# MariusFurter/WeightedSampling.jl

Measured on NVIDIA B200. Metric: particle_updates_per_sec, higher is better.
Workload: dtype f64

## Files before the change

weightedsampling.jl_b200/csrc/ws_internal.h:

```cpp
#pragma once
#include <cuda_runtime.h>
#include <stdint.h>
#include "ws_vm.cuh"
#include "ws_mailbox.cuh"

#ifndef WS_VM_BLOCK
#define WS_VM_BLOCK 128
#endif
#ifndef WS_VM_P
#define WS_VM_P 3
#endif
#ifndef WS_VM_MINB
#define WS_VM_MINB 5
#endif
#define WS_VM_MAX_IO 24
#define WS_VM_MAX_CKPT 16
#define WS_VM_MAX_OPS 96
#define WS_VM_MAX_REGS ((192 * 1024) / (WS_VM_BLOCK * WS_VM_P * 8))
#define WS_SCAN_BLOCK 256
#define WS_SCAN_ITEMS 8
#define WS_SCAN_TILE (32 * WS_SCAN_ITEMS)
#define WS_CDF_TILE (WS_SCAN_BLOCK * WS_SCAN_ITEMS)
#define WS_GATHER_MAX_PLANES 32
#define WS_HEAVY_TILE_SLOTS 32768
#define WS_MAX_PARTIALS 4096

struct WsLse {
    double m, S, Q;
};

struct WsReduceOut {
    double m, S, Q;
    double lse;
    double ess_perc;
    double log_mean_w;
    int32_t do_resample;
    int32_t pad;
};

struct WsVmProgram {
    int64_t n;
    int64_t particle_offset;
    int32_t n_ops, n_loads, n_stores, n_regs;
    const double* load_ptr[WS_VM_MAX_IO];
    double* store_ptr[WS_VM_MAX_IO];
    uint8_t load_reg[WS_VM_MAX_IO];
    uint8_t store_reg[WS_VM_MAX_IO];
    const int32_t* ancestors;
    uint32_t load_gather;
    int32_t logw_mode;
    double* logw;
    double logw_base;
    WsLse* partials;
    int32_t n_expect;
    uint8_t expect_reg[8];
    const WsReduceOut* red;
    double* expect_partials;
    int32_t n_ckpt;
    uint8_t ckpt_pc[WS_VM_MAX_CKPT];
    WsLse* ckpt_partials;
    double* logw_out;
    WsRng rng;
    WsOp ops[WS_VM_MAX_OPS];
};

struct WsScanParams {
    const double* logw;
    int32_t mode;
    int32_t scheme;
    const WsReduceOut* red;
    int32_t gate;
    int32_t pad;
    int64_t n;
    int64_t n_slots;
    unsigned long long cdf_offset;
    const unsigned long long* all_tot;
    int32_t rank;
    int32_t pad2;
    int32_t slot_base;
    int32_t last_rank;
    int32_t* bounds;
    unsigned long long* total;
    uint64_t seed, stream;
    const double* replay_u;
    const double* sorted_u;
    int32_t* ancestors;
    unsigned long long* tile_words;
    unsigned long long* cdf_local;
    unsigned int* tile_counter;
    double fx_scale;
    int32_t fx_shift;
    int32_t mn_shift;
    unsigned long long* mn_tile_off;
    unsigned long long* mn_block_local;
    unsigned long long* mn_total;
    unsigned long long* n_clamped;
    unsigned int* heavy_count;
    int32_t* heavy_F;
};

struct WsGatherParams {
    int64_t n;
    const int32_t* ancestors;
    int32_t n_planes;
    int32_t pad;
    const double* src[WS_GATHER_MAX_PLANES];
    double* dst[WS_GATHER_MAX_PLANES];
};

#define WS_COMPOSE_MAX_CHAIN 24
struct WsComposeParams {
    int64_t n;
    int64_t n_rows;
    int32_t n_chain;
    int32_t pad;
    const int32_t* chain[WS_COMPOSE_MAX_CHAIN];
};

cudaError_t ws_launch_vm(const WsVmProgram& P, int grid, cudaStream_t s);
cudaError_t ws_launch_reduce_logw(const double* logw, int64_t n, WsLse* partials, int grid, cudaStream_t s);
cudaError_t ws_launch_finalize(const WsLse* partials, int n_partials, int k, int64_t n_global, double ess_perc_min,
                               WsReduceOut* out, unsigned long long* ties, cudaStream_t s);
#define WS_SMALL_N 4096
cudaError_t ws_launch_resample_small(const WsScanParams& P, const WsLse* partials, int n_partials, double ess_perc_min, WsReduceOut* out,
                                     unsigned long long* ties, int do_finalize, cudaStream_t s);
void ws_scan_set_scale(WsScanParams& P);
size_t ws_scan_words(int64_t n);
cudaError_t ws_launch_scan_search(const WsScanParams& P, int grid, cudaStream_t s);
cudaError_t ws_launch_spacings(const WsScanParams& P, cudaStream_t s);
cudaError_t ws_launch_cdf(const WsScanParams& P, cudaStream_t s);
cudaError_t ws_launch_bounds(const WsScanParams& P, cudaStream_t s);
cudaError_t ws_launch_search(const WsScanParams& P, cudaStream_t s);
cudaError_t ws_launch_finalize_global(const double* all_msq, int n_ranks, int64_t n_global, double ess_perc_min,
                                      WsReduceOut* out, cudaStream_t s, unsigned long long* ties = nullptr);
cudaError_t ws_launch_finalize_mbox(const WsLse* partials, int n_partials, int64_t n_global, double ess_perc_min, WsReduceOut* out,
                                    double* all_msq, unsigned long long* ties, const WsMailbox& M, cudaStream_t s);
cudaError_t ws_launch_cdf_tiles(const WsScanParams& P, cudaStream_t s);
cudaError_t ws_launch_offsets_bounds_mbox(const WsScanParams& P, const WsMailbox& M, unsigned long long* all_tot, const unsigned long long* xmine,
                                          int xw, unsigned long long* xall, cudaStream_t s);
cudaError_t ws_launch_barrier_mbox(const WsMailbox& M, cudaStream_t s);
cudaError_t ws_launch_gather(const WsGatherParams& P, int grid, cudaStream_t s);
cudaError_t ws_launch_fill(double* dst, double v, int64_t n, int grid, cudaStream_t s);
cudaError_t ws_launch_exp_norm(const double* logw, const WsReduceOut* red, double* w, int64_t n, int grid,
                               cudaStream_t s);
cudaError_t ws_launch_sumsq(const double* w, int64_t n, double* partials, int grid, cudaStream_t s);
cudaError_t ws_launch_local_ancestors(int32_t* anc, int64_t n, const int32_t* anc_self, int64_t self_lo, int64_t self_hi,
                                      int64_t spare_base, int grid, cudaStream_t s);
cudaError_t ws_launch_patch_ancestors(int32_t* anc, int64_t n, int64_t self_lo, int64_t self_hi, int64_t spare_base, cudaStream_t s);
struct WsTracedPlane {
    const double* src;
    double* dst;
    int64_t level;
};
cudaError_t ws_launch_trace_rows(const int32_t* anc, int64_t m, const int32_t* const* chain, int n_levels, int64_t n_rows, int32_t* rows,
                                 cudaStream_t s);
cudaError_t ws_launch_push_traced(const WsTracedPlane* planes, int n_planes, int64_t m, const int32_t* rows, cudaStream_t s);
cudaError_t ws_launch_gather_rows(const double* src, const int64_t* idx, int64_t n_idx, double* dst, cudaStream_t s);
cudaError_t ws_launch_compose(const WsComposeParams& P, int32_t* out, const int32_t* start, cudaStream_t s);
cudaError_t ws_launch_compose_rows(const WsComposeParams& P, int64_t* out, const int64_t* start, cudaStream_t s);
int ws_vm_sl_grid(const WsVmProgram& P);
int ws_vm_max_grid(int n_regs, int n_loads, int n_ops, int sm_count, int n_ckpt = 0);
int ws_vm_smem_bytes(int n_regs, int n_loads, int n_ops, int n_ckpt = 0);
cudaError_t ws_kernels_init(int device);
```

weightedsampling.jl_b200/csrc/ws_kernels.cu:

```cuda
#include "ws_internal.h"

static int g_sm_count = 148;

__device__ __forceinline__ void lse_push(WsLse& a, double l) {
    if (l == -INFINITY) return;
    if (l > a.m) {
        double sc = ws_exp_nonpos(a.m - l);
        a.S = a.S * sc + 1.0;
        a.Q = a.Q * sc * sc + 1.0;
        a.m = l;
    } else {
        double e = ws_exp_nonpos(l - a.m);
        a.S += e;
        a.Q += e * e;
    }
}

template <int K>
__device__ __forceinline__ void lse_push_many(WsLse& a, const double (&l)[K], const bool (&live)[K]) {
    double mx = -INFINITY;
#pragma unroll
    for (int j = 0; j < K; ++j)
        if (live[j]) mx = fmax(mx, l[j]);
    if (mx > a.m) {
// ... 11 lines not shown
        }
    }
}

__device__ __forceinline__ WsLse lse_combine(const WsLse& a, const WsLse& b) {
    if (b.m == -INFINITY) return a;
    if (a.m == -INFINITY) return b;
    WsLse r;
    r.m = fmax(a.m, b.m);
    double ea = ws_exp_nonpos(a.m - r.m), eb = ws_exp_nonpos(b.m - r.m);
    r.S = a.S * ea + b.S * eb;
    r.Q = a.Q * ea * ea + b.Q * eb * eb;
    return r;
}

__device__ __forceinline__ WsLse lse_shfl_down(const WsLse& a, int delta) {
    WsLse r;
    r.m = __shfl_down_sync(0xffffffffu, a.m, delta);
    r.S = __shfl_down_sync(0xffffffffu, a.S, delta);
    r.Q = __shfl_down_sync(0xffffffffu, a.Q, delta);
    return r;
}

template <int BLOCK>
__device__ __forceinline__ WsLse lse_block_reduce(WsLse v, WsLse* warp_scratch ) {
#pragma unroll
    for (int d = 16; d > 0; d >>= 1) v = lse_combine(v, lse_shfl_down(v, d));
    const int lane = threadIdx.x & 31, warp = threadIdx.x >> 5;
    if (lane == 0) warp_scratch[warp] = v;
    __syncthreads();
    if (warp == 0) {
        WsLse t;
        if (lane < BLOCK / 32) {
            t = warp_scratch[lane];
        } else {
            t.m = -INFINITY;
            t.S = 0.0;
            t.Q = 0.0;
        }
#pragma unroll
        for (int d = 16; d > 0; d >>= 1) t = lse_combine(t, lse_shfl_down(t, d));
        v = t;
    }
    return v;
}

template <int BLOCK>
__device__ __forceinline__ WsLse lse_block_combine(const WsLse* __restrict__ partials, int n_partials, WsLse* warp_scratch ) {
    WsLse part;
    part.m = -INFINITY;
    part.S = 0.0;
    part.Q = 0.0;
    for (int i = threadIdx.x; i < n_partials; i += BLOCK) part = lse_combine(part, partials[i]);
    return lse_block_reduce<BLOCK>(part, warp_scratch);
}

__device__ __forceinline__ WsLse lse_combine_ranks(const double* msq, int n_ranks) {
    WsLse tot;
    tot.m = -INFINITY;
    tot.S = 0.0;
    tot.Q = 0.0;
    for (int r = 0; r < n_ranks; ++r) {
        WsLse v;
        v.m = msq[3 * r + 0];
        v.S = msq[3 * r + 1];
        v.Q = msq[3 * r + 2];
        tot = lse_combine(tot, v);
    }
    return tot;
}

__device__ __forceinline__ void ws_decide(const WsLse& tot, int64_t n_global, double ess_perc_min, WsReduceOut* out,
                                          unsigned long long* ties) {
    out->m = tot.m;
    out->S = tot.S;
    out->Q = tot.Q;
    const double lse = tot.m + log(tot.S);
    out->lse = lse;
    const double nn = (double)n_global;
    out->ess_perc = (tot.S * tot.S) / (nn * tot.Q);
    out->log_mean_w = lse - log(nn);
    out->do_resample = (out->ess_perc < ess_perc_min) ? 1 : 0;
    if (ties != nullptr && fabs(out->ess_perc - ess_perc_min) <= 8.0 * 2.220446049250313e-16 * fabs(ess_perc_min)) atomicAdd(ties, 1ull);
}

__device__ __forceinline__ void ws_cp_async8(double* smem_dst, const double* gsrc) {
    const unsigned d = (unsigned)__cvta_generic_to_shared(smem_dst);
    asm volatile("cp.async.ca.shared.global [%0], [%1], 8;" ::"r"(d), "l"(gsrc) : "memory");
}
__device__ __forceinline__ void ws_cp_async16(void* smem_dst, const void* gsrc) {
    const unsigned d = (unsigned)__cvta_generic_to_shared(smem_dst);
    asm volatile("cp.async.cg.shared.global [%0], [%1], 16;" ::"r"(d), "l"(gsrc) : "memory");
}
__device__ __forceinline__ void ws_cp_async_commit() { asm volatile("cp.async.commit_group;" ::: "memory"); }
__device__ __forceinline__ void ws_cp_async_wait_all() { asm volatile("cp.async.wait_group 0;" ::: "memory"); }

template <bool STAGED, bool CKPT = false>
__global__ void __launch_bounds__(WS_VM_BLOCK, WS_VM_MINB) ws_vm_kernel(const __grid_constant__ WsVmProgram P) {
    extern __shared__ __align__(16) double ws_vm_smem[];
    __shared__ WsLse warp_scratch[WS_VM_BLOCK / 32];
    double* R = ws_vm_smem + threadIdx.x;
    constexpr int RS = WS_VM_P * WS_VM_BLOCK;
    double* const stage = R + P.n_regs * RS;
    WsDop* const dops = reinterpret_cast<WsDop*>(ws_vm_smem + (P.n_regs + (STAGED ? P.n_loads : 0)) * RS);
    for (int t = threadIdx.x; t < P.n_ops; t += WS_VM_BLOCK) dops[t] = ws_decode_op<WS_VM_BLOCK, WS_VM_P>(P.ops[t]);
    double* const ck = reinterpret_cast<double*>(dops + P.n_ops) + threadIdx.x;
    for (int c = 0; CKPT && c < P.n_ckpt; ++c) {
        ck[(c * 3 + 0) * WS_VM_BLOCK] = -INFINITY;
        ck[(c * 3 + 1) * WS_VM_BLOCK] = 0.0;
        ck[(c * 3 + 2) * WS_VM_BLOCK] = 0.0;
    }
    __syncthreads();

    WsLse part;
    part.m = -INFINITY;
    part.S = 0.0;
    part.Q = 0.0;
    double esum[8];
#pragma unroll
    for (int k = 0; k < 8; ++k) esum[k] = 0.0;
    double red_m = 0.0, red_invS = 0.0;
    if (P.n_expect > 0) {
        red_m = P.red->m;
        red_invS = 1.0 / P.red->S;
    }

    constexpr int TILE = WS_VM_BLOCK * WS_VM_P;
    const int n = (int)P.n;
    const int n_tiles = (n + TILE - 1) / TILE;
    const bool fired = (P.logw_mode != 3) || P.red->do_resample != 0;
    const int lmode = (P.logw_mode == 3) ? (fired ? 2 : 1) : P.logw_mode;
    const double lbase = (P.logw_mode == 3) ? P.red->log_mean_w : P.logw_base;
    const bool any_gather = P.load_gather != 0u && fired;

    auto tile_index = [&](int tile, int j) -> int {
        const int i = tile * TILE + (int)threadIdx.x + j * WS_VM_BLOCK;
        return i < n ? i : n - 1;
    };
    auto issue_stage = [&](int tile, const int (&anc)[WS_VM_P]) {
        for (int k = 0; k < P.n_loads; ++k) {
            const bool g = any_gather && ((P.load_gather >> k) & 1u);
            const double* __restrict__ ptr = P.load_ptr[k];
            double* dst = stage + k * RS;
#pragma unroll
            for (int j = 0; j < WS_VM_P; ++j)
                ws_cp_async8(dst + j * WS_VM_BLOCK, ptr + (unsigned)(g ? anc[j] : tile_index(tile, j)));
        }
        ws_cp_async_commit();
    };

    int anc_next[WS_VM_P];
    if (STAGED) {
        const int t0 = blockIdx.x, t1 = blockIdx.x + gridDim.x;
        if (t0 < n_tiles) {
            int a0[WS_VM_P];
#pragma unroll
            for (int j = 0; j < WS_VM_P; ++j) a0[j] = any_gather ? __ldg(P.ancestors + tile_index(t0, j)) : 0;
            issue_stage(t0, a0);
        }
#pragma unroll
        for (int j = 0; j < WS_VM_P; ++j) anc_next[j] = (any_gather && t1 < n_tiles) ? __ldg(P.ancestors + tile_index(t1, j)) : 0;
    }

    for (int tile = blockIdx.x; tile < n_tiles; tile += gridDim.x) {
        int idx[WS_VM_P];
        bool live[WS_VM_P];
// ... 98 lines not shown
            const double* srcr = R + (int)P.store_reg[k] * RS;
            double* __restrict__ ptr = P.store_ptr[k];
#pragma unroll
            for (int j = 0; j < WS_VM_P; ++j)
                if (live[j]) ptr[(unsigned)idx[j]] = srcr[j * WS_VM_BLOCK];
        }
        if (P.logw_mode != 0) {
            double lw[WS_VM_P];
#pragma unroll
            for (int j = 0; j < WS_VM_P; ++j) {
                lw[j] = (CKPT ? lw_run[j] : (lmode == 1 ? lw_old[j] : lbase)) + acc[j];
                if (live[j]) (CKPT && P.logw_out != nullptr ? P.logw_out : P.logw)[(unsigned)idx[j]] = lw[j];
            }
            lse_push_many<WS_VM_P>(part, lw, live);
        }
        if (P.n_expect > 0) {
#pragma unroll
            for (int j = 0; j < WS_VM_P; ++j) {
                if (live[j]) {
                    const double w = ws_exp_nonpos(lw_old[j] - red_m) * red_invS;
#pragma unroll
                    for (int k = 0; k < 8; ++k) {
                        if (k < P.n_expect) esum[k] += w * R[(int)P.expect_reg[k] * RS + j * WS_VM_BLOCK];
                    }
                }
            }
        }
    }

    if (P.logw_mode != 0 && P.partials != nullptr) {
        WsLse tot = lse_block_reduce<WS_VM_BLOCK>(part, warp_scratch);
        if (threadIdx.x == 0) P.partials[blockIdx.x] = tot;
    }
    for (int c = 0; CKPT && c < P.n_ckpt; ++c) {
        WsLse st;
        st.m = ck[(c * 3 + 0) * WS_VM_BLOCK];
        st.S = ck[(c * 3 + 1) * WS_VM_BLOCK];
        st.Q = ck[(c * 3 + 2) * WS_VM_BLOCK];
        __syncthreads();
        WsLse tot = lse_block_reduce<WS_VM_BLOCK>(st, warp_scratch);
        if (threadIdx.x == 0) P.ckpt_partials[(size_t)c * gridDim.x + blockIdx.x] = tot;
    }
    if (P.n_expect > 0) {
        __shared__ double esc[WS_VM_BLOCK / 32][8];
        const int lane = threadIdx.x & 31, warp = threadIdx.x >> 5;
#pragma unroll
        for (int k = 0; k < 8; ++k) {
            double v = esum[k];
#pragma unroll
            for (int d = 16; d > 0; d >>= 1) v += __shfl_down_sync(0xffffffffu, v, d);
            if (lane == 0) esc[warp][k] = v;
        }
        __syncthreads();
        if (threadIdx.x < 8 && threadIdx.x < P.n_expect) {
            double v = 0.0;
            for (int w = 0; w < WS_VM_BLOCK / 32; ++w) v += esc[w][threadIdx.x];
            P.expect_partials[(size_t)blockIdx.x * P.n_expect + threadIdx.x] = v;
        }
    }
}

#include "ws_vm_sl.cuh"
#ifndef WS_SL_P
#define WS_SL_P 4
#endif
#ifndef WS_SL_MINB
#define WS_SL_MINB 3
#endif
template <class Sig, int PP>
__global__ void __launch_bounds__(WS_VM_BLOCK, WS_SL_MINB) ws_vm_sl_kernel(const __grid_constant__ WsVmProgram P) {
    extern __shared__ __align__(16) double ws_vm_smem[];
    __shared__ WsLse warp_scratch[WS_VM_BLOCK / 32];
    constexpr int RS = PP * WS_VM_BLOCK;
    constexpr int TILE = WS_VM_BLOCK * PP;
    constexpr int NL = Sig::n_loads, NS = Sig::n_stores;
    double* const stage = ws_vm_smem + threadIdx.x;

    WsLse part;
    part.m = -INFINITY;
    part.S = 0.0;
    part.Q = 0.0;
    const int n = (int)P.n;
    const int n_tiles = (n + TILE - 1) / TILE;
    const bool fired = (P.logw_mode != 3) || P.red->do_resample != 0;
    const int lmode = (P.logw_mode == 3) ? (fired ? 2 : 1) : P.logw_mode;
    const double lbase = (P.logw_mode == 3) ? P.red->log_mean_w : P.logw_base;
    const bool any_gather = P.load_gather != 0u && fired;

    auto tile_index = [&](int tile, int j) -> int {
        const int i = tile * TILE + (int)threadIdx.x + j * WS_VM_BLOCK;
        return i < n ? i : n - 1;
    };
    auto issue_stage = [&](int tile, const int (&anc)[PP]) {
#pragma unroll
        for (int k = 0; k < NL; ++k) {
            const bool g = any_gather && ((P.load_gather >> k) & 1u);
            const double* __restrict__ ptr = P.load_ptr[k];
#pragma unroll
            for (int j = 0; j < PP; ++j)
                ws_cp_async8(stage + k * RS + j * WS_VM_BLOCK, ptr + (unsigned)(g ? anc[j] : tile_index(tile, j)));
        }
        ws_cp_async_commit();
    };

    WsSlConsts<Sig> K;
    ws_sl_load_consts<Sig>(K, P, std::make_integer_sequence<int, Sig::n_ops>{});
    const bool replay = P.rng.replay_n != nullptr || P.rng.replay_u != nullptr || P.rng.replay_e != nullptr;

    int anc_next[PP];
    {
        const int t0 = blockIdx.x, t1 = blockIdx.x + gridDim.x;
        if (t0 < n_tiles) {
            int a0[PP];
#pragma unroll
            for (int j = 0; j < PP; ++j) a0[j] = any_gather ? __ldg(P.ancestors + tile_index(t0, j)) : 0;
            issue_stage(t0, a0);
        }
#pragma unroll
        for (int j = 0; j < PP; ++j) anc_next[j] = (any_gather && t1 < n_tiles) ? __ldg(P.ancestors + tile_index(t1, j)) : 0;
    }

    for (int tile = blockIdx.x; tile < n_tiles; tile += gridDim.x) {
        int idx[PP];
        bool live[PP];
        uint64_t particle[PP];
        const int first = tile * TILE + (int)threadIdx.x;
#pragma unroll
        for (int j = 0; j < PP; ++j) {
            const int i = first + j * WS_VM_BLOCK;
            live[j] = i < n;
            idx[j] = live[j] ? i : n - 1;
            particle[j] = (uint64_t)(P.particle_offset + (int64_t)idx[j]);
        }
        double R[Sig::n_regs * PP];
        if (NL > 0) {
            ws_cp_async_wait_all();
            ws_sl_loads<Sig, PP, WS_VM_BLOCK>(R, stage, std::make_integer_sequence<int, NL>{});
            const int tn = tile + gridDim.x, tnn = tn + gridDim.x;
            if (tn < n_tiles) issue_stage(tn, anc_next);
            if (any_gather && tnn < n_tiles) {
#pragma unroll
                for (int j = 0; j < PP; ++j) anc_next[j] = __ldg(P.ancestors + tile_index(tnn, j));
            }
        }
        double lw_old[PP];
#pragma unroll
        for (int j = 0; j < PP; ++j) lw_old[j] = 0.0;
        if (lmode == 1) {
#pragma unroll
            for (int j = 0; j < PP; ++j) lw_old[j] = P.logw[(unsigned)idx[j]];
        }

        double acc[PP];
#pragma unroll
        for (int j = 0; j < PP; ++j) acc[j] = 0.0;
        ws_sl_run<Sig, PP>(R, acc, P, K, replay, particle, std::make_integer_sequence<int, Sig::n_ops>{});

        ws_sl_stores<Sig, PP, WS_VM_BLOCK>(R, P, (unsigned)first, live, std::make_integer_sequence<int, NS>{});
        if (P.logw_mode != 0) {
            double lw[PP];
#pragma unroll
            for (int j = 0; j < PP; ++j) {
                lw[j] = (lmode == 1 ? lw_old[j] : lbase) + acc[j];
                if (live[j]) P.logw[(unsigned)first + j * WS_VM_BLOCK] = lw[j];
            }
            lse_push_many<PP>(part, lw, live);
        }
    }
    if (P.logw_mode != 0 && P.partials != nullptr) {
        WsLse tot = lse_block_reduce<WS_VM_BLOCK>(part, warp_scratch);
        if (threadIdx.x == 0) P.partials[blockIdx.x] = tot;
    }
}

#ifndef WS_SLCK_N
#define WS_SLCK_N 8
#endif
#ifndef WS_SLCK_P
#define WS_SLCK_P 2
#endif
#ifndef WS_SLCK_MINB
#define WS_SLCK_MINB 4
#endif
template <class Sig, int PP, int NCK>
__global__ void __launch_bounds__(WS_VM_BLOCK, WS_SLCK_MINB) ws_vm_sl_ckpt_kernel(const __grid_constant__ WsVmProgram P) {
    extern __shared__ __align__(16) double ws_vm_smem[];
    __shared__ WsLse warp_scratch[WS_VM_BLOCK / 32];
    __shared__ double kc[NCK][Sig::n_ops][3];
    constexpr int RS = PP * WS_VM_BLOCK;
    constexpr int TILE = WS_VM_BLOCK * PP;
// ... 27 lines not shown
        for (int k = 0; k < NL; ++k) {
            const bool g = any_gather && ((P.load_gather >> k) & 1u);
            const double* __restrict__ ptr = P.load_ptr[k];
#pragma unroll
            for (int j = 0; j < PP; ++j) {
                const int i = tile_index(tile, j);
                ws_cp_async8(stage + k * RS + j * WS_VM_BLOCK, ptr + (unsigned)(g ? __ldg(P.ancestors + i) : i));
            }
        }
        ws_cp_async_commit();
    };
    if ((int)blockIdx.x < n_tiles) issue_stage(blockIdx.x);
    for (int tile = blockIdx.x; tile < n_tiles; tile += gridDim.x) {
        bool live[PP];
        uint64_t particle[PP];
        const int first = tile * TILE + (int)threadIdx.x;
#pragma unroll
        for (int j = 0; j < PP; ++j) {
            const int i = first + j * WS_VM_BLOCK;
            live[j] = i < n;
            particle[j] = (uint64_t)(P.particle_offset + (int64_t)(live[j] ? i : n - 1));
        }
        double R[Sig::n_regs * PP];
        ws_cp_async_wait_all();
        ws_sl_loads<Sig, PP, WS_VM_BLOCK>(R, stage, std::make_integer_sequence<int, NL>{});
        if (tile + (int)gridDim.x < n_tiles) issue_stage(tile + gridDim.x);
        double lw[PP];
#pragma unroll
        for (int j = 0; j < PP; ++j) lw[j] = lmode == 1 ? P.logw[(unsigned)tile_index(tile, j)] : lbase;
#pragma unroll
        for (int c = 0; c < NCK; ++c) {
            if (c < reps) {
                WsSlConsts<Sig> K;
#pragma unroll
                for (int i = 0; i < Sig::n_ops; ++i) {
                    K.k[i][0] = kc[c][i][0];
                    K.k[i][1] = kc[c][i][1];
                    K.k[i][2] = kc[c][i][2];
                }
                double acc[PP];
#pragma unroll
                for (int j = 0; j < PP; ++j) acc[j] = 0.0;
                ws_sl_run_at<Sig, PP>(R, acc, P, P.ops + c * Sig::n_ops, K, particle, std::make_integer_sequence<int, Sig::n_ops>{});
#pragma unroll
                for (int j = 0; j < PP; ++j) lw[j] += acc[j];
                lse_push_many<PP>(st[c], lw, live);
            }
        }
        double* const lout = P.logw_out != nullptr ? P.logw_out : P.logw;
#pragma unroll
        for (int j = 0; j < PP; ++j)
            if (live[j]) lout[(unsigned)first + j * WS_VM_BLOCK] = lw[j];
    }
#pragma unroll
    for (int c = 0; c < NCK; ++c) {
        if (c < reps) {
            __syncthreads();
            WsLse tot = lse_block_reduce<WS_VM_BLOCK>(st[c], warp_scratch);
            if (threadIdx.x == 0) {
                P.ckpt_partials[(size_t)c * gridDim.x + blockIdx.x] = tot;
                if (c == reps - 1 && P.partials != nullptr) P.partials[blockIdx.x] = tot;
            }
        }
    }
}
static bool ws_slck_ok(const WsVmProgram& P) {
    return P.n_ckpt > 0 && P.n_expect == 0 && (P.logw_mode == 1 || P.logw_mode == 2) && ws_sl_matches_repeated<WsSigLinregObs>(P, WS_SLCK_N);
}
static int ws_slck_grid(const WsVmProgram& P) {
    constexpr int TILE = WS_VM_BLOCK * WS_SLCK_P;
    const int64_t tiles = (P.n + TILE - 1) / TILE;
    const int grid = (int)(tiles < (int64_t)g_sm_count * WS_SLCK_MINB ? tiles : (int64_t)g_sm_count * WS_SLCK_MINB);
    return grid < 1 ? 1 : grid;
}

static bool g_vm_interp_only = false;
template <class Sig>
static cudaError_t ws_launch_vm_sl(const WsVmProgram& P, cudaStream_t s) {
    constexpr int TILE = WS_VM_BLOCK * WS_SL_P;
    const int64_t tiles = (P.n + TILE - 1) / TILE;
    int grid = (int)(tiles < (int64_t)g_sm_count * WS_SL_MINB ? tiles : (int64_t)g_sm_count * WS_SL_MINB);
    if (grid < 1) grid = 1;
    const int smem = (Sig::n_loads > 0 ? Sig::n_loads : 1) * TILE * (int)sizeof(double);
    ws_vm_sl_kernel<Sig, WS_SL_P><<<grid, WS_VM_BLOCK, smem, s>>>(P);
    return cudaGetLastError();
}
int ws_vm_sl_grid(const WsVmProgram& P) {
    if (!g_vm_interp_only && P.n_ckpt != 0 && ws_slck_ok(P)) return ws_slck_grid(P);
    if (g_vm_interp_only || P.n_ckpt != 0 || ws_sl_find(P) < 0) return 0;
    constexpr int TILE = WS_VM_BLOCK * WS_SL_P;
    const int64_t tiles = (P.n + TILE - 1) / TILE;
    int grid = (int)(tiles < (int64_t)g_sm_count * WS_SL_MINB ? tiles : (int64_t)g_sm_count * WS_SL_MINB);
    return grid < 1 ? 1 : grid;
}

static bool ws_vm_staged(int n_regs, int n_loads) {
    return n_loads > 0 && (size_t)(n_regs + n_loads) * WS_VM_BLOCK * WS_VM_P * sizeof(double) <= (size_t)200 * 1024;
}
int ws_vm_smem_bytes(int n_regs, int n_loads, int n_ops, int n_ckpt) {
    const int rows = (n_regs < 1 ? 1 : n_regs) + (ws_vm_staged(n_regs < 1 ? 1 : n_regs, n_loads) ? n_loads : 0);
    return rows * WS_VM_BLOCK * WS_VM_P * (int)sizeof(double) + n_ops * (int)sizeof(WsDop) + n_ckpt * 3 * WS_VM_BLOCK * (int)sizeof(double);
}

int ws_vm_max_grid(int n_regs, int n_loads, int n_ops, int sm_count, int n_ckpt) {
    const int smem = ws_vm_smem_bytes(n_regs, n_loads, n_ops, n_ckpt) + 1024;
    int per_sm = (227 * 1024) / smem;
    if (per_sm > WS_VM_MINB) per_sm = WS_VM_MINB;
    if (per_sm < 1) per_sm = 1;
    return per_sm * sm_count;
}

cudaError_t ws_launch_vm(const WsVmProgram& P, int grid, cudaStream_t s) {
    if (!g_vm_interp_only && P.n_ckpt == 0) {
        switch (ws_sl_find(P)) {
#define WS_SL_CASE(idx, Sig) \
    case idx: return ws_launch_vm_sl<Sig>(P, s);
            WS_SL_SIGS(WS_SL_CASE)
#undef WS_SL_CASE
            default: break;
        }
    }
    if (!g_vm_interp_only && P.n_ckpt != 0 && ws_slck_ok(P)) {
        constexpr int smem_ck = WsSigLinregObs::n_loads * WS_VM_BLOCK * WS_SLCK_P * (int)sizeof(double);
        ws_vm_sl_ckpt_kernel<WsSigLinregObs, WS_SLCK_P, WS_SLCK_N><<<ws_slck_grid(P), WS_VM_BLOCK, smem_ck, s>>>(P);
        return cudaGetLastError();
    }
    const int smem = ws_vm_smem_bytes(P.n_regs, P.n_loads, P.n_ops, P.n_ckpt);
    if (P.n_ckpt > 0) {
        if (ws_vm_staged(P.n_regs, P.n_loads)) ws_vm_kernel<true, true><<<grid, WS_VM_BLOCK, smem, s>>>(P);
        else ws_vm_kernel<false, true><<<grid, WS_VM_BLOCK, smem, s>>>(P);
    } else if (ws_vm_staged(P.n_regs, P.n_loads)) ws_vm_kernel<true><<<grid, WS_VM_BLOCK, smem, s>>>(P);
    else ws_vm_kernel<false><<<grid, WS_VM_BLOCK, smem, s>>>(P);
    return cudaGetLastError();
}

__global__ void __launch_bounds__(256) ws_reduce_logw_kernel(const double* __restrict__ logw, int64_t n,
                                                             WsLse* __restrict__ partials) {
    __shared__ WsLse warp_scratch[8];
    WsLse part;
    part.m = -INFINITY;
    part.S = 0.0;
    part.Q = 0.0;
    const int64_t stride = (int64_t)gridDim.x * 256;
    for (int64_t i = (int64_t)blockIdx.x * 256 + threadIdx.x; i < n; i += stride) lse_push(part, __ldg(logw + i));
    WsLse tot = lse_block_reduce<256>(part, warp_scratch);
    if (threadIdx.x == 0) partials[blockIdx.x] = tot;
}

cudaError_t ws_launch_reduce_logw(const double* logw, int64_t n, WsLse* partials, int grid, cudaStream_t s) {
    ws_reduce_logw_kernel<<<grid, 256, 0, s>>>(logw, n, partials);
    return cudaGetLastError();
}

__global__ void __launch_bounds__(256) ws_finalize_kernel(const WsLse* __restrict__ partials, int n_partials,
                                                          int64_t n_global, double ess_perc_min,
                                                          WsReduceOut* __restrict__ out, unsigned long long* ties) {
    __shared__ WsLse warp_scratch[8];
    const WsLse tot = lse_block_combine<256>(partials + (size_t)blockIdx.x * n_partials, n_partials, warp_scratch);
    if (threadIdx.x == 0) ws_decide(tot, n_global, ess_perc_min, out + blockIdx.x, ties);
}

cudaError_t ws_launch_finalize(const WsLse* partials, int n_partials, int k, int64_t n_global, double ess_perc_min,
                               WsReduceOut* out, unsigned long long* ties, cudaStream_t s) {
    ws_finalize_kernel<<<k, 256, 0, s>>>(partials, n_partials, n_global, ess_perc_min, out, ties);
    return cudaGetLastError();
}

__global__ void ws_finalize_global_kernel(const double* __restrict__ all_msq, int n_ranks, int64_t n_global,
// ... 60 lines not shown
    asm volatile("ld.relaxed.gpu.global.u64 %0, [%1];" : "=l"(v) : "l"(p) : "memory");
    return v;
}
__device__ __forceinline__ void st_relaxed_u64(unsigned long long* p, unsigned long long v) {
    asm volatile("st.relaxed.gpu.global.u64 [%0], %1;" ::"l"(p), "l"(v) : "memory");
}

struct SlotUniform {
    int scheme;
    uint64_t seed, stream;
    const double* replay;
    double r0;
    int64_t cached_blk;
    ws_u32x4 cached;
    __device__ __forceinline__ double operator()(int64_t k) {
        if (scheme == 1) return r0;
        if (replay != nullptr) return replay[k];
        const int64_t blk = k >> 1;
        if (blk != cached_blk) {
            cached = ws_philox4x32_10((uint64_t)blk, stream, seed);
            cached_blk = blk;
        }
        return (k & 1) ? ws_u01(cached.z, cached.w) : ws_u01(cached.x, cached.y);
    }
};

__device__ __forceinline__ int64_t ws_count_sorted_le(const double* __restrict__ us, int64_t n, double C) {
    int64_t lo = 0, hi = n;
    while (lo < hi) {
        int64_t mid = (lo + hi) >> 1;
        if (__ldg(us + mid) <= C) lo = mid + 1; else hi = mid;
    }
    return lo;
}

__device__ __forceinline__ int64_t ws_F(const WsScanParams& P, double C, double inv_n, SlotUniform& su) {
    if (P.sorted_u != nullptr) return ws_count_sorted_le(P.sorted_u, P.n_slots, C);
    return ws_count_slots_le(C, P.n_slots, inv_n, su);
}

#define WS_TILE_GROUP 32
#define WS_EXPAND_CHUNK 512
#ifndef WS_EXPAND_LANE
#define WS_EXPAND_LANE 12
#endif
#define WS_DIRECT_MAX 8
#define WS_WARPS_PER_CTA (WS_SCAN_BLOCK / 32)
#define WS_MN_MAX_WINDOWS 64
#define WS_RBUF_SLOTS 512

__device__ __forceinline__ void ws_slot_split(unsigned long long C, unsigned int n, int sh, unsigned int& k, unsigned int& frac) {
    const unsigned long long T = sh >= 0 ? (C >> sh) : (C << (-sh));
    const unsigned long long k64 = T >> 32;
    k = (k64 >= (unsigned long long)n) ? n : (unsigned int)k64;
    frac = (unsigned int)T;
}
__device__ __forceinline__ unsigned int ws_slot_word(const ws_u32x4& b, unsigned int k) {
    const unsigned int j = k & 3u;
    return j == 0u ? b.x : (j == 1u ? b.y : (j == 2u ? b.z : b.w));
}
__device__ __forceinline__ int ws_F_int(unsigned long long C, unsigned int n, int sh, unsigned int rmask, int scheme, unsigned int r0,
                                        uint64_t seed, uint64_t stream) {
    unsigned int k, frac;
    ws_slot_split(C, n, sh, k, frac);
    if (k >= n) return (int)n;
    unsigned int r;
    if (scheme == 1) {
        r = r0;
    } else {
        r = ws_slot_word(ws_philox4x32_10((uint64_t)(k >> 2), stream, seed), k);
    }
    return (int)k + ((r & rmask) <= frac ? 1 : 0);
}

#ifndef WS_CDF_ASYNC
#define WS_CDF_ASYNC 0
#endif
#ifndef WS_CDF_MINB
#define WS_CDF_MINB 4
#endif
#ifndef WS_CDF_GRID
#define WS_CDF_GRID 4
#endif
__global__ void __launch_bounds__(WS_SCAN_BLOCK, WS_CDF_MINB) ws_cdf_tiles_kernel(const __grid_constant__ WsScanParams P) {
    if (P.gate != 0 && P.red->do_resample == 0) return;
    __shared__ unsigned long long warp_tot[2][WS_SCAN_BLOCK / 32];
    int parity = 0;
    const int lane = threadIdx.x & 31, warp = threadIdx.x >> 5;
    const int n = (int)P.n;
    const int n_tiles = (n + WS_CDF_TILE - 1) / WS_CDF_TILE;
    double m = 0.0, Sden = 1.0;
    if (P.mode == 0) {
        m = P.red->m;
        Sden = P.red->S;
    }
    const double rS = 1.0 / Sden;
    const double uniform_w = 1.0 / (double)P.n_slots;
#if WS_CDF_ASYNC
    __shared__ __align__(16) double2 lbuf_all[WS_SCAN_ITEMS / 2][WS_SCAN_BLOCK];
    double2* const lbuf = &lbuf_all[0][threadIdx.x];
    auto request = [&](int tile) {
        if (P.mode != 2 && (tile + 1) * WS_CDF_TILE <= n) {
            const double2* p2 = reinterpret_cast<const double2*>(P.logw + (size_t)tile * WS_CDF_TILE + threadIdx.x * WS_SCAN_ITEMS);
#pragma unroll
            for (int k = 0; k < WS_SCAN_ITEMS / 2; ++k) ws_cp_async16(lbuf + k * WS_SCAN_BLOCK, p2 + k);
        }
        ws_cp_async_commit();
    };
    if ((int)blockIdx.x < n_tiles) request(blockIdx.x);
    for (int tile = blockIdx.x; tile < n_tiles; tile += gridDim.x) {
        const int item0 = tile * WS_CDF_TILE + threadIdx.x * WS_SCAN_ITEMS;
        unsigned long long q[WS_SCAN_ITEMS];
        if (P.mode == 2) {
#pragma unroll
            for (int k = 0; k < WS_SCAN_ITEMS; ++k) q[k] = (item0 + k < n) ? ws_w_to_fxs(uniform_w, P.fx_scale) : 0ull;
        } else {
            double l[WS_SCAN_ITEMS];
            ws_cp_async_wait_all();
            if ((tile + 1) * WS_CDF_TILE <= n) {
#pragma unroll
                for (int k = 0; k < WS_SCAN_ITEMS / 2; ++k) {
                    const double2 v = lbuf[k * WS_SCAN_BLOCK];
                    l[2 * k] = v.x;
                    l[2 * k + 1] = v.y;
                }
            } else {
#pragma unroll
                for (int k = 0; k < WS_SCAN_ITEMS; ++k) l[k] = (item0 + k < n) ? __ldg(P.logw + item0 + k) : -INFINITY;
            }
            if (tile + (int)gridDim.x < n_tiles) request(tile + gridDim.x);
            if (P.mode == 0) {
#pragma unroll
                for (int k = 0; k < WS_SCAN_ITEMS; ++k)
                    q[k] = __double2ull_rn(ws_div_pos(ws_exp_nonpos_or0(l[k] - m), Sden, rS) * P.fx_scale);
            } else {
#pragma unroll
                for (int k = 0; k < WS_SCAN_ITEMS; ++k) q[k] = (item0 + k < n) ? ws_w_to_fxs(l[k], P.fx_scale) : 0ull;
            }
        }
#else
    auto load_tile = [&](int tile, double (&l)[WS_SCAN_ITEMS]) {
        const int item0 = tile * WS_CDF_TILE + threadIdx.x * WS_SCAN_ITEMS;
        if (item0 + WS_SCAN_ITEMS <= n) {
            const double2* p2 = reinterpret_cast<const double2*>(P.logw + item0);
#pragma unroll
            for (int k = 0; k < WS_SCAN_ITEMS / 2; ++k) {
                double2 v = __ldg(p2 + k);
                l[2 * k] = v.x;
                l[2 * k + 1] = v.y;
            }
        } else {
#pragma unroll
            for (int k = 0; k < WS_SCAN_ITEMS; ++k) l[k] = (item0 + k < n) ? __ldg(P.logw + item0 + k) : -INFINITY;
        }
    };
    double l[WS_SCAN_ITEMS];
#pragma unroll
    for (int k = 0; k < WS_SCAN_ITEMS; ++k) l[k] = -INFINITY;
    if (P.mode != 2 && (int)blockIdx.x < n_tiles) load_tile(blockIdx.x, l);
    for (int tile = blockIdx.x; tile < n_tiles; tile += gridDim.x) {
        const int item0 = tile * WS_CDF_TILE + threadIdx.x * WS_SCAN_ITEMS;
        unsigned long long q[WS_SCAN_ITEMS];
        if (P.mode == 2) {
#pragma unroll
            for (int k = 0; k < WS_SCAN_ITEMS; ++k) q[k] = (item0 + k < n) ? ws_w_to_fxs(uniform_w, P.fx_scale) : 0ull;
        } else {
            if (P.mode == 0) {
#pragma unroll
                for (int k = 0; k < WS_SCAN_ITEMS; ++k)
                    q[k] = __double2ull_rn(ws_div_pos(ws_exp_nonpos_or0(l[k] - m), Sden, rS) * P.fx_scale);
            } else {
#pragma unroll
                for (int k = 0; k < WS_SCAN_ITEMS; ++k) q[k] = (item0 + k < n) ? ws_w_to_fxs(l[k], P.fx_scale) : 0ull;
            }
            if (tile + (int)gridDim.x < n_tiles) load_tile(tile + gridDim.x, l);
        }
#endif
#pragma unroll
        for (int k = 1; k < WS_SCAN_ITEMS; ++k) q[k] += q[k - 1];
        const unsigned long long thread_total = q[WS_SCAN_ITEMS - 1];
        unsigned long long incl = thread_total;
#pragma unroll
        for (int d = 1; d < 32; d <<= 1) {
            unsigned long long t = __shfl_up_sync(0xffffffffu, incl, d);
            if (lane >= d) incl += t;
        }
        unsigned long long* const wt = warp_tot[parity];
        parity ^= 1;
        if (lane == 31) wt[warp] = incl;
        __syncthreads();
        unsigned long long t8 = lane < WS_SCAN_BLOCK / 32 ? wt[lane] : 0ull;
#pragma unroll
        for (int d = 1; d < WS_SCAN_BLOCK / 32; d <<= 1) {
            const unsigned long long t = __shfl_up_sync(0xffffffffu, t8, d);
            if (lane >= d) t8 += t;
        }
        const unsigned long long tile_agg = __shfl_sync(0xffffffffu, t8, WS_SCAN_BLOCK / 32 - 1);
        unsigned long long warp_excl = __shfl_sync(0xffffffffu, t8, (warp + 31) & 31);
        if (warp == 0) warp_excl = 0ull;
        const unsigned long long thread_excl = warp_excl + (incl - thread_total);
        if (item0 + WS_SCAN_ITEMS <= n) {
            ulonglong2* dst = reinterpret_cast<ulonglong2*>(P.cdf_local + item0);
#pragma unroll
            for (int k = 0; k < WS_SCAN_ITEMS / 2; ++k) dst[k] = make_ulonglong2(thread_excl + q[2 * k], thread_excl + q[2 * k + 1]);
        } else {
#pragma unroll
            for (int k = 0; k < WS_SCAN_ITEMS; ++k)
                if (item0 + k < n) P.cdf_local[item0 + k] = thread_excl + q[k];
        }
        if (threadIdx.x == 0) P.tile_words[tile] = tile_agg;
    }
}

#define WS_OFF_ITEMS 8
__device__ __forceinline__ void ws_scan_words_cta(unsigned long long* __restrict__ words, const int n_tiles, unsigned long long* total_out) {
    __shared__ unsigned long long warp_tot[32];
    __shared__ unsigned long long s_carry;
    const int lane = threadIdx.x & 31, warp = threadIdx.x >> 5;
    if (threadIdx.x == 0) s_carry = 0ull;
    __syncthreads();
    for (int base = 0; base < n_tiles; base += 1024 * WS_OFF_ITEMS) {
        const int i0 = base + threadIdx.x * WS_OFF_ITEMS;
        unsigned long long v[WS_OFF_ITEMS];
#pragma unroll
        for (int k = 0; k < WS_OFF_ITEMS; ++k) v[k] = (i0 + k < n_tiles) ? words[i0 + k] : 0ull;
        unsigned long long thread_total = 0ull;
#pragma unroll
        for (int k = 0; k < WS_OFF_ITEMS; ++k) thread_total += v[k];
        unsigned long long incl = thread_total;
#pragma unroll
        for (int d = 1; d < 32; d <<= 1) {
            unsigned long long t = __shfl_up_sync(0xffffffffu, incl, d);
            if (lane >= d) incl += t;
        }
        if (lane == 31) warp_tot[warp] = incl;
        __syncthreads();
        unsigned long long warp_excl = 0ull, total = 0ull;
#pragma unroll
        for (int w = 0; w < 32; ++w) {
            const unsigned long long t = warp_tot[w];
            if (w < warp) warp_excl += t;
            total += t;
        }
        const unsigned long long carry = s_carry;
        unsigned long long run = carry + warp_excl + (incl - thread_total);
#pragma unroll
        for (int k = 0; k < WS_OFF_ITEMS; ++k) {
            if (i0 + k < n_tiles) words[i0 + k] = run;
            run += v[k];
        }
        __syncthreads();
        if (threadIdx.x == 0) s_carry = carry + total;
        __syncthreads();
    }
    if (threadIdx.x == 0 && total_out != nullptr) *total_out = s_carry;
}
__global__ void __launch_bounds__(1024) ws_cdf_offsets_kernel(const __grid_constant__ WsScanParams P) {
    if (P.gate != 0 && P.red->do_resample == 0) return;
    ws_scan_words_cta(P.tile_words, (int)((P.n + WS_CDF_TILE - 1) / WS_CDF_TILE), P.total);
}
__device__ __forceinline__ void ws_cdf_group_offsets_body(const WsScanParams& P) {
    if (threadIdx.x == 0 && P.heavy_count != nullptr) *P.heavy_count = 0u;
    if (P.gate != 0 && P.red->do_resample == 0) return;
    const int n_tiles = (int)((P.n + WS_CDF_TILE - 1) / WS_CDF_TILE);
    const int n_groups = (n_tiles + WS_TILE_GROUP - 1) / WS_TILE_GROUP;
    unsigned long long* const grp = P.tile_words + n_tiles;
    const int lane = threadIdx.x & 31, warp = threadIdx.x >> 5;
    for (int g = warp; g < n_groups; g += 32) {
        const int idx = g * WS_TILE_GROUP + lane;
        unsigned long long v = idx < n_tiles ? P.tile_words[idx] : 0ull;
#pragma unroll
        for (int d = 16; d > 0; d >>= 1) v += __shfl_xor_sync(0xffffffffu, v, d);
        if (lane == 0) grp[g] = v;
    }
    __syncthreads();
    ws_scan_words_cta(grp, n_groups, P.total);
}
__global__ void __launch_bounds__(1024) ws_cdf_group_offsets_kernel(const __grid_constant__ WsScanParams P) { ws_cdf_group_offsets_body(P); }
__device__ __forceinline__ unsigned long long ws_tile_offset(const WsScanParams& P, const int n_tiles, const int ct, const int lane) {
    const int g = ct / WS_TILE_GROUP, idx = g * WS_TILE_GROUP + lane;
    unsigned long long v = idx < ct ? __ldg(P.tile_words + idx) : 0ull;
    if (lane == 31) v = __ldg(P.tile_words + n_tiles + g);
#pragma unroll
    for (int d = 16; d > 0; d >>= 1) v += __shfl_xor_sync(0xffffffffu, v, d);
    return v;
}

__device__ __forceinline__ unsigned long long ws_mn_threshold(unsigned long long C, unsigned long long S_total) {
    const unsigned long long lo = C * S_total, hi = __umul64hi(C, S_total);
    return (hi << 3) | (lo >> 61);
}
__device__ __forceinline__ unsigned long long ws_mn_block_prefix(const WsScanParams& P, int b) {
    return __ldg(P.mn_tile_off + b / (WS_CDF_TILE / WS_SCAN_TILE)) + __ldg(P.mn_block_local + b);
}
__device__ __forceinline__ int ws_mn_find_block(const WsScanParams& P, unsigned long long T) {
    constexpr int BPT = WS_CDF_TILE / WS_SCAN_TILE;
    const int n_all = (int)P.n_slots + 1;
    const int n_tiles = (n_all + WS_CDF_TILE - 1) / WS_CDF_TILE, n_blocks = (n_all + WS_SCAN_TILE - 1) / WS_SCAN_TILE;
    int lo = 0, hi = n_tiles - 1;
    while (lo < hi) {
        const int mid = (lo + hi + 1) >> 1;
        if (__ldg(P.mn_tile_off + mid) <= T) lo = mid; else hi = mid - 1;
    }
    const unsigned long long base = __ldg(P.mn_tile_off + lo);
    int b = lo * BPT;
    const int b_end = min(b + BPT, n_blocks);
    for (int j = b + 1; j < b_end; ++j)
        if (base + __ldg(P.mn_block_local + j) <= T) b = j;
    return b;
}
__device__ __forceinline__ int ws_F_mn(const WsScanParams& P, unsigned long long C) {
    const int ns = (int)P.n_slots;
    const unsigned long long T = ws_mn_threshold(C, *P.mn_total);
    const int b = ws_mn_find_block(P, T);
    unsigned long long S = ws_mn_block_prefix(P, b);
    int k = b * WS_SCAN_TILE;
    const int k_end = min(k + WS_SCAN_TILE, ns);
    while (k < k_end) {
        S += ws_spacing_of_slot((uint64_t)k, P.mn_shift, P.seed, P.stream);
        if (S > T) break;
        ++k;
    }
    return k;
}

__global__ void __launch_bounds__(WS_SCAN_BLOCK) ws_spacing_tiles_kernel(const __grid_constant__ WsScanParams P) {
    if (P.gate != 0 && P.red->do_resample == 0) return;
    __shared__ unsigned long long warp_tot[WS_SCAN_BLOCK / 32];
    const int lane = threadIdx.x & 31, warp = threadIdx.x >> 5;
    const int n_all = (int)P.n_slots + 1;
    const int n_tiles = (n_all + WS_CDF_TILE - 1) / WS_CDF_TILE;
    for (int tile = blockIdx.x; tile < n_tiles; tile += gridDim.x) {
        const int k0 = tile * WS_CDF_TILE + threadIdx.x * WS_SCAN_ITEMS;
        unsigned long long sum = 0ull;
#pragma unroll
        for (int j = 0; j < WS_SCAN_ITEMS / 2; ++j) {
            const int k = k0 + 2 * j;
            if (k < n_all) {
                const ws_u32x4 r = ws_philox4x32_10((uint64_t)(k >> 1), P.stream, P.seed);
                sum += ws_spacing_fx(r.x, r.y, P.mn_shift);
                if (k + 1 < n_all) sum += ws_spacing_fx(r.z, r.w, P.mn_shift);
            }
        }
#pragma unroll
        for (int d = 16; d > 0; d >>= 1) sum += __shfl_xor_sync(0xffffffffu, sum, d);
        __syncthreads();
        if (lane == 0) warp_tot[warp] = sum;
        __syncthreads();
        unsigned long long excl = 0ull, agg = 0ull;
#pragma unroll
        for (int w = 0; w < WS_SCAN_BLOCK / 32; ++w) {
            const unsigned long long t = warp_tot[w];
            if (w < warp) excl += t;
            agg += t;
        }
        const int b = tile * (WS_CDF_TILE / WS_SCAN_TILE) + warp;
        if (lane == 0 && b * WS_SCAN_TILE < n_all) P.mn_block_local[b] = excl;
        if (threadIdx.x == 0) P.mn_tile_off[tile] = agg;
    }
}

// ... 408 lines not shown
            }
            int excl = __shfl_up_sync(0xffffffffu, incl, 1);
            if (lane == 0) excl = -1;
#pragma unroll
            for (int j = 0; j < PL; ++j) mk[j] = max(mk[j], excl);
            const int p0 = lane * PL;
            if (p0 >= pad && p0 + PL <= W) {
#pragma unroll
                for (int j = 0; j < Q; ++j)
                    *reinterpret_cast<int4*>(dst + p0 + 4 * j) = make_int4(mk[4 * j], mk[4 * j + 1], mk[4 * j + 2], mk[4 * j + 3]);
            } else {
#pragma unroll
                for (int j = 0; j < PL; ++j)
                    if (p0 + j >= pad && p0 + j < W) dst[p0 + j] = mk[j];
            }
        }
        __syncwarp();
        return;
    }
    bool has_big = false;
    {
        int lo = f_prev;
#pragma unroll
        for (int k = 0; k < WS_SCAN_ITEMS; ++k) {
            if (f[k] - lo > WS_DIRECT_MAX) has_big = true;
            lo = f[k];
        }
    }
    const unsigned big_mask = __ballot_sync(0xffffffffu, has_big);
    for (int chunk = fstart; chunk < fend; chunk += WS_EXPAND_CHUNK) {
        const int chunk_end = min(chunk + WS_EXPAND_CHUNK, fend);
        {
            int lo = f_prev;
#pragma unroll
            for (int k = 0; k < WS_SCAN_ITEMS; ++k) {
                const int hi = f[k];
                if (hi - lo <= WS_DIRECT_MAX) {
                    const int a = max(lo, chunk), e = min(hi, chunk_end);
                    for (int pos = a; pos < e; ++pos) out_s[pos - chunk] = item0 + k;
                }
                lo = hi;
            }
        }
        unsigned bm = big_mask;
        while (bm != 0u) {
            const int src = __ffs(bm) - 1;
            bm &= bm - 1u;
            int lo = __shfl_sync(0xffffffffu, f_prev, src);
#pragma unroll
            for (int k = 0; k < WS_SCAN_ITEMS; ++k) {
                const int hi = __shfl_sync(0xffffffffu, f[k], src);
                if (hi - lo > WS_DIRECT_MAX) {
                    const int a = max(lo, chunk), e = min(hi, chunk_end);
                    const int anc = tile_base + src * WS_SCAN_ITEMS + k;
                    for (int pos = a + lane; pos < e; pos += 32) out_s[pos - chunk] = anc;
                }
                lo = hi;
            }
        }
        __syncwarp();
        for (int pos = chunk + lane; pos < chunk_end; pos += 32) P.ancestors[pos - slot_base] = out_s[pos - chunk];
        __syncwarp();
    }
}

#ifndef WS_SEARCH_ASYNC
#define WS_SEARCH_ASYNC 1
#endif
#ifndef WS_SEARCH_MINB
#define WS_SEARCH_MINB 3
#endif
#ifndef WS_SEARCH_GRID
#define WS_SEARCH_GRID 3
#endif
__device__ __forceinline__ bool ws_gate_closed_identity(const WsScanParams& P) {
    if (P.gate == 0 || P.red->do_resample != 0) return false;
    const int64_t stride = (int64_t)gridDim.x * blockDim.x;
    for (int64_t i = (int64_t)blockIdx.x * blockDim.x + threadIdx.x; i < P.n; i += stride) P.ancestors[i] = (int32_t)i;
    return true;
}
#define WS_SEARCH_SMEM_BYTES ((WS_WARPS_PER_CTA * WS_RBUF_SLOTS + WS_CDF_TILE) * 8)
template <bool EXACT_FP, bool MN, bool SHR>
__global__ void __launch_bounds__(WS_SCAN_BLOCK, WS_SEARCH_MINB) ws_search_kernel(const __grid_constant__ WsScanParams P) {
    if (ws_gate_closed_identity(P)) return;

    extern __shared__ __align__(16) unsigned long long search_smem[];
    static_assert(WS_RBUF_SLOTS * 8 >= (WS_EXPAND_CHUNK + 128) * 4 && (WS_RBUF_SLOTS * 8) % 16 == 0, "window too small for the offspring staging");
    const int lane = threadIdx.x & 31, warp = threadIdx.x >> 5;
    unsigned long long* const rbuf = search_smem + warp * WS_RBUF_SLOTS;
    ulonglong2* const cbuf = reinterpret_cast<ulonglong2*>(search_smem + WS_WARPS_PER_CTA * WS_RBUF_SLOTS + warp * WS_SCAN_TILE) + lane;

    const unsigned long long cdf_offset = ws_cdf_offset(P);
    WsSearchCtx X;
    ws_search_setup(P, X);
    const int n = X.n;
    const int n_tiles = (n + WS_SCAN_TILE - 1) / WS_SCAN_TILE;
    const int n_ctiles = (n + WS_CDF_TILE - 1) / WS_CDF_TILE;
    const int warps_total = gridDim.x * WS_WARPS_PER_CTA;

#if WS_SEARCH_ASYNC
    unsigned long long ow = 0ull, pw = 0ull;
    auto request = [&](int tile) {
        const int tile_base = tile * WS_SCAN_TILE;
        const int ct = tile_base / WS_CDF_TILE;
        if (tile_base + WS_SCAN_TILE <= n) {
            const ulonglong2* p2 = reinterpret_cast<const ulonglong2*>(P.cdf_local + tile_base + lane * WS_SCAN_ITEMS);
#pragma unroll
            for (int k = 0; k < WS_SCAN_ITEMS / 2; ++k) ws_cp_async16(cbuf + k * 32, p2 + k);
        }
        ws_cp_async_commit();
        const int idx = (ct / WS_TILE_GROUP) * WS_TILE_GROUP + lane;
        ow = idx < ct ? __ldg(P.tile_words + idx) : 0ull;
        if (lane == 31) ow = __ldg(P.tile_words + n_ctiles + ct / WS_TILE_GROUP);
        pw = (lane == 0 && tile_base % WS_CDF_TILE != 0) ? __ldg(P.cdf_local + tile_base - 1) : 0ull;
    };
    static_assert(WS_EXPAND_CHUNK * 4 + WS_RING_BLOCKS * 16 <= WS_RBUF_SLOTS * 8 && 32 * WS_EXPAND_LANE <= WS_EXPAND_CHUNK,
                  "the ring and the offspring staging share a window");
    WsRing ring{reinterpret_cast<uint4*>(rbuf + WS_EXPAND_CHUNK / 2), 0u, 0u};
    const int per_warp = (n_tiles + warps_total - 1) / warps_total;
    int tile = (blockIdx.x * WS_WARPS_PER_CTA + warp) * per_warp;
    const int tile_end = min(tile + per_warp, n_tiles);
    if (tile < tile_end) request(tile);
    for (; tile < tile_end; ++tile) {
        const int tile_base = tile * WS_SCAN_TILE;
        const int item0 = tile_base + lane * WS_SCAN_ITEMS;
        unsigned long long C[WS_SCAN_ITEMS];
        ws_cp_async_wait_all();
        if (tile_base + WS_SCAN_TILE <= n) {
#pragma unroll
            for (int k = 0; k < WS_SCAN_ITEMS / 2; ++k) {
                const ulonglong2 v = cbuf[k * 32];
                C[2 * k] = v.x;
                C[2 * k + 1] = v.y;
            }
        } else {
#pragma unroll
            for (int k = 0; k < WS_SCAN_ITEMS; ++k) C[k] = (item0 + k < n) ? __ldg(P.cdf_local + item0 + k) : 0ull;
        }
        unsigned long long off = ow;
        const unsigned long long pl = pw;
        if (tile + 1 < tile_end) request(tile + 1);
#pragma unroll
        for (int d = 16; d > 0; d >>= 1) off += __shfl_xor_sync(0xffffffffu, off, d);
        off += cdf_offset;
        if (tile_base + WS_SCAN_TILE <= n) {
#pragma unroll
            for (int k = 0; k < WS_SCAN_ITEMS; ++k) C[k] += off;
        } else {
#pragma unroll
            for (int k = 0; k < WS_SCAN_ITEMS; ++k) C[k] = (item0 + k < n) ? off + C[k] : 0ull;
        }
        ws_search_warp_tile<EXACT_FP, MN, SHR>(P, X, rbuf, lane, tile_base, C, off + pl, tile != 0,
                                               WS_INTERIOR_FAST && tile_base + WS_SCAN_TILE < n, &ring);
    }
#else
    for (int tile = blockIdx.x * WS_WARPS_PER_CTA + warp; tile < n_tiles; tile += warps_total) {
        const int tile_base = tile * WS_SCAN_TILE;
        const int item0 = tile_base + lane * WS_SCAN_ITEMS;
        const int ct = tile_base / WS_CDF_TILE;
        const unsigned long long offset = cdf_offset + ws_tile_offset(P, n_ctiles, ct, lane);

        unsigned long long C[WS_SCAN_ITEMS];
        if (item0 + WS_SCAN_ITEMS <= n) {
            const ulonglong2* p2 = reinterpret_cast<const ulonglong2*>(P.cdf_local + item0);
#pragma unroll
            for (int k = 0; k < WS_SCAN_ITEMS / 2; ++k) {
// ... 74 lines not shown
    for (int k = 1; k < WS_SCAN_ITEMS; ++k) q[k] += q[k - 1];
    const unsigned long long thread_total = q[WS_SCAN_ITEMS - 1];
    unsigned long long incl = thread_total;
#pragma unroll
    for (int d = 1; d < 32; d <<= 1) {
        const unsigned long long t = __shfl_up_sync(0xffffffffu, incl, d);
        if (lane >= d) incl += t;
    }
    if (lane == 31) warp_tot[warp] = incl;
    __syncthreads();
    unsigned long long warp_excl = 0ull, tile_agg = 0ull;
#pragma unroll
    for (int w = 0; w < WS_WARPS_PER_CTA; ++w) {
        const unsigned long long t = warp_tot[w];
        if (w < warp) warp_excl += t;
        tile_agg += t;
    }

    if (tile == 0) {
        if (threadIdx.x == 0) {
            st_relaxed_u64(P.tile_words, (WS_TILE_INCL << 62) | tile_agg);
            s_prefix = 0ull;
        }
    } else {
        if (threadIdx.x == 0) st_relaxed_u64(P.tile_words + tile, (WS_TILE_AGG << 62) | tile_agg);
        unsigned long long excl = 0ull;
        int look = tile - 1;
        while (true) {
            const int idx = look - (int)threadIdx.x;
            unsigned long long word;
            do {
                word = (idx >= 0) ? ld_relaxed_u64(P.tile_words + idx) : (WS_TILE_INCL << 62);
            } while (__any_sync(0xffffffffu, (word >> 62) == 0ull));
            const unsigned incl_mask = __ballot_sync(0xffffffffu, (word >> 62) == WS_TILE_INCL);
            const int first = incl_mask != 0u ? __ffs(incl_mask) - 1 : 31;
            unsigned long long v = (lane <= first) ? (word & WS_FXS_MASK) : 0ull;
#pragma unroll
            for (int d = 16; d > 0; d >>= 1) v += __shfl_xor_sync(0xffffffffu, v, d);
            __syncthreads();
            if (lane == 0) {
                lb_sum[warp] = v;
                lb_found[warp] = incl_mask != 0u ? 1 : 0;
            }
            __syncthreads();
            bool found = false;
#pragma unroll
            for (int w = 0; w < WS_WARPS_PER_CTA; ++w) {
                if (!found) {
                    excl += lb_sum[w];
                    found = lb_found[w] != 0;
                }
            }
            if (found) break;
            look -= WS_SCAN_BLOCK;
        }
        if (threadIdx.x == 0) {
            st_relaxed_u64(P.tile_words + tile, (WS_TILE_INCL << 62) | (excl + tile_agg));
            s_prefix = excl;
        }
    }
    __syncthreads();
    const unsigned long long prefix = P.cdf_offset + s_prefix;

    unsigned long long C[WS_SCAN_ITEMS];
    const unsigned long long thread_excl = prefix + warp_excl + (incl - thread_total);
#pragma unroll
    for (int k = 0; k < WS_SCAN_ITEMS; ++k) C[k] = (item0 + k < n) ? thread_excl + q[k] : 0ull;
    const int warp_base = tile * WS_CDF_TILE + warp * WS_SCAN_TILE;
    if (warp_base < n) ws_search_warp_tile<EXACT_FP, false>(P, X, win_all[warp], lane, warp_base, C, prefix + warp_excl, warp_base != 0);
}

#define WS_CHAIN_GROUP WS_TILE_GROUP
#ifndef WS_CHAIN_MINB
#define WS_CHAIN_MINB 3
#endif
#ifndef WS_CHAIN_MAXREG
#define WS_CHAIN_MAXREG 80
#endif
#define WS_CHAIN_CNT_SHIFT 40
#define WS_CHAIN_PART_MASK ((1ull << WS_CHAIN_CNT_SHIFT) - 1ull)
#define WS_CHAIN_SMEM_BYTES(BLOCK) ((((BLOCK) / 32) * WS_RBUF_SLOTS + 2 * (BLOCK) * WS_SCAN_ITEMS) * 8)
#define WS_CHAIN_MIN_TILE (32 * WS_SCAN_ITEMS)

size_t ws_scan_words(int64_t n) {
    const int64_t n_tiles = (n + WS_CHAIN_MIN_TILE - 1) / WS_CHAIN_MIN_TILE;
    const int64_t n_groups = (n_tiles + WS_CHAIN_GROUP - 1) / WS_CHAIN_GROUP;
    return (size_t)(n_tiles + 3 * n_groups + 2);
}

template <bool EXACT_FP, int BLOCK>
__global__ void __maxnreg__(WS_CHAIN_MAXREG) ws_chain_kernel(const __grid_constant__ WsScanParams P) {
    constexpr int TILE = BLOCK * WS_SCAN_ITEMS;
    constexpr int WARPS = BLOCK / 32;
    constexpr int GRP_WARP = WARPS > 1 ? 1 : 0;
    if (ws_gate_closed_identity(P)) return;
    extern __shared__ __align__(16) unsigned long long chain_smem[];
    __shared__ unsigned long long warp_tot[WARPS];
    __shared__ unsigned long long s_wexcl[WARPS];
    __shared__ unsigned long long lb_part[2];
    __shared__ int s_tile;
    const int tid = threadIdx.x, lane = tid & 31, warp = tid >> 5;
    unsigned long long* const win = chain_smem + warp * WS_RBUF_SLOTS;
    ulonglong2* const stash = reinterpret_cast<ulonglong2*>(chain_smem + WARPS * WS_RBUF_SLOTS) + tid;
    double2* const lbuf = reinterpret_cast<double2*>(chain_smem + WARPS * WS_RBUF_SLOTS + TILE) + tid;
    const int n = (int)P.n;
    const int n_tiles = (n + TILE - 1) / TILE;
    const int n_groups = (n_tiles + WS_CHAIN_GROUP - 1) / WS_CHAIN_GROUP;
    unsigned long long* const grp_lo = P.tile_words + n_tiles;
    unsigned long long* const grp_hi = grp_lo + n_groups;
    unsigned long long* const grp_incl = grp_hi + n_groups;
    WsSearchCtx X;
    ws_search_setup(P, X);
    double m = 0.0, Sden = 1.0;
    if (P.mode == 0) {
        m = P.red->m;
        Sden = P.red->S;
    }
    const double rS = 1.0 / Sden;
    const double uniform_w = 1.0 / (double)P.n_slots;
    auto prefetch = [&](int tile) {
        if (P.mode != 2 && tile < n_tiles && (tile + 1) * TILE <= n) {
            const double2* p2 = reinterpret_cast<const double2*>(P.logw + (size_t)tile * TILE + tid * WS_SCAN_ITEMS);
#pragma unroll
            for (int k = 0; k < WS_SCAN_ITEMS / 2; ++k) ws_cp_async16(lbuf + k * BLOCK, p2 + k);
        }
        ws_cp_async_commit();
    };
    if (tid == 0) s_tile = (int)atomicAdd(P.tile_counter, 1u);
    __syncthreads();
    int t1 = s_tile;
    prefetch(t1);
    __syncthreads();
    int t0 = -1;
    while (true) {
        const bool have1 = t1 < n_tiles;
        if (tid == 0) s_tile = (int)atomicAdd(P.tile_counter, 1u);
        unsigned long long lbt = 0ull, lbw0 = 0ull, lbw1 = 0ull, lbw2 = 0ull;
        if (t0 >= 0) {
            const int g0 = t0 / WS_CHAIN_GROUP;
            if (warp == 0) {
                const int idx = g0 * WS_CHAIN_GROUP + lane;
                if (idx < t0) lbt = ld_relaxed_u64(P.tile_words + idx);
            }
            if (warp == GRP_WARP) {
                const int gi = g0 - 1 - lane;
                if (gi >= 0) {
                    lbw0 = ld_relaxed_u64(grp_incl + gi);
                    lbw1 = ld_relaxed_u64(grp_lo + gi);
                    lbw2 = ld_relaxed_u64(grp_hi + gi);
                }
            }
        }
        unsigned long long q[WS_SCAN_ITEMS];
        unsigned long long incl = 0ull, thread_total = 0ull;
        if (have1) {
            const int base = t1 * TILE;
            const int item0 = base + tid * WS_SCAN_ITEMS;
            if (P.mode == 2) {
                const unsigned long long qu = ws_w_to_fxs(uniform_w, P.fx_scale);
#pragma unroll
                for (int k = 0; k < WS_SCAN_ITEMS; ++k) q[k] = (item0 + k < n) ? qu : 0ull;
            } else {
                double l[WS_SCAN_ITEMS];
                if (base + TILE <= n) {
                    ws_cp_async_wait_all();
#pragma unroll
                    for (int k = 0; k < WS_SCAN_ITEMS / 2; ++k) {
                        const double2 v = lbuf[k * BLOCK];
                        l[2 * k] = v.x;
                        l[2 * k + 1] = v.y;
// ... 152 lines not shown
        if (threadIdx.x == 0) {
            ws_decide(tot, P.n_slots, ess_perc_min, out, ties);
            __threadfence_block();
        }
        __syncthreads();
    }
    if (threadIdx.x == 0) {
        s_fire = (P.gate == 0 || out->do_resample != 0) ? 1 : 0;
        s_carry = 0ull;
    }
    __syncthreads();
    const int n = (int)P.n, ns = (int)P.n_slots;
    if (!s_fire) {
        for (int i = threadIdx.x; i < n; i += 256) P.ancestors[i] = i;
        return;
    }
    const double m = out->m, Sden = out->S, rS = 1.0 / out->S;
    const int sh = P.fx_shift - 32;
    const unsigned int rmask = sh >= 0 ? 0xFFFFFFFFu : ~((1u << (-sh)) - 1u);
    unsigned int r0 = 0u;
    if (P.scheme == 1) r0 = ws_philox4x32_10(0ull, P.stream, P.seed).x;
    for (int base = 0; base < n; base += 256 * WS_SCAN_ITEMS) {
        const int item0 = base + threadIdx.x * WS_SCAN_ITEMS;
        unsigned long long q[WS_SCAN_ITEMS];
#pragma unroll
        for (int k = 0; k < WS_SCAN_ITEMS; ++k) {
            const int i = item0 + k;
            q[k] = (i < n) ? ws_w_to_fxs(ws_div_pos(ws_exp_nonpos(P.logw[i] - m), Sden, rS), P.fx_scale) : 0ull;
        }
#pragma unroll
        for (int k = 1; k < WS_SCAN_ITEMS; ++k) q[k] += q[k - 1];
        const unsigned long long thread_total = q[WS_SCAN_ITEMS - 1];
        unsigned long long incl = thread_total;
#pragma unroll
        for (int d = 1; d < 32; d <<= 1) {
            const unsigned long long t = __shfl_up_sync(0xffffffffu, incl, d);
            if (lane >= d) incl += t;
        }
        __syncthreads();
        if (lane == 31) warp_tot[warp] = incl;
        __syncthreads();
        unsigned long long warp_excl = 0ull, chunk_tot = 0ull;
#pragma unroll
        for (int w = 0; w < 8; ++w) {
            const unsigned long long t = warp_tot[w];
            if (w < warp) warp_excl += t;
            chunk_tot += t;
        }
        const unsigned long long excl = s_carry + warp_excl + (incl - thread_total);
#pragma unroll
        for (int k = 0; k < WS_SCAN_ITEMS; ++k) {
            const int i = item0 + k;
            if (i < n) {
                int fk = ws_F_int(excl + q[k], (unsigned int)ns, sh, rmask, P.scheme == 1 ? 1 : 0, r0, P.seed, P.stream);
                if (i == n - 1) {
                    if (fk < ns) atomicAdd(P.n_clamped, (unsigned long long)(ns - fk));
                    fk = ns;
                }
                Fs[i] = fk;
            }
        }
        __syncthreads();
        if (threadIdx.x == 0) s_carry += chunk_tot;
    }
    __syncthreads();
    for (int j = threadIdx.x; j < ns; j += 256) {
        int lo = 0, hi = n - 1;
        while (lo < hi) {
            const int mid = (lo + hi) >> 1;
            if (Fs[mid] > j) hi = mid; else lo = mid + 1;
        }
        P.ancestors[j] = lo;
    }
}

cudaError_t ws_launch_resample_small(const WsScanParams& P, const WsLse* partials, int n_partials, double ess_perc_min, WsReduceOut* out,
                                     unsigned long long* ties, int do_finalize, cudaStream_t s) {
    ws_resample_small_kernel<<<1, 256, 0, s>>>(P, partials, n_partials, ess_perc_min, out, ties, do_finalize,
                                               reinterpret_cast<int32_t*>(P.cdf_local));
    return cudaGetLastError();
}

__global__ void __launch_bounds__(256) ws_expand_heavy_kernel(const __grid_constant__ WsScanParams P) {
    if (P.gate != 0 && P.red->do_resample == 0) return;
    __shared__ int32_t Fs[WS_SCAN_TILE];
    const unsigned int n_heavy = *P.heavy_count;
    for (unsigned int h = 0; h < n_heavy; ++h) {
        const int32_t* src = P.heavy_F + (size_t)h * (WS_SCAN_TILE + 2);
        __syncthreads();
        for (int k = threadIdx.x; k < WS_SCAN_TILE; k += 256) Fs[k] = src[k];
        __syncthreads();
        const int64_t fstart = (int64_t)src[WS_SCAN_TILE];
        const int64_t tile_base = (int64_t)src[WS_SCAN_TILE + 1] * WS_SCAN_TILE;
        const int64_t fend = (int64_t)Fs[WS_SCAN_TILE - 1];
        const int64_t len = fend - fstart;
        const int64_t per = (len + gridDim.x - 1) / gridDim.x;
        const int64_t a = fstart + (int64_t)blockIdx.x * per;
        const int64_t e = (a + per < fend) ? a + per : fend;
        for (int64_t j = a + threadIdx.x; j < e; j += 256) {
            int lo = 0, hi = WS_SCAN_TILE - 1;
            while (lo < hi) {
                const int mid = (lo + hi) >> 1;
                if ((int64_t)Fs[mid] > j) hi = mid; else lo = mid + 1;
            }
            P.ancestors[j - P.slot_base] = (int32_t)(tile_base + lo);
        }
    }
}

static int g_fx_extra_bits = 0;
void ws_scan_set_scale(WsScanParams& P) {
    const bool exact_fp = P.replay_u != nullptr || P.sorted_u != nullptr;
    int shift = 61;
    {
        int bits = 0;
        while (((int64_t)1 << bits) < P.n_slots + 1) ++bits;
        P.mn_shift = 60 - bits;
    }
    if (!exact_fp && P.scheme != 2) {
        int bits = 0;
        while (((int64_t)1 << bits) < P.n_slots) ++bits;
        shift = 61 - bits - g_fx_extra_bits;
        if (shift < 24) shift = 24;
    }
    P.fx_shift = shift;
    P.fx_scale = (exact_fp || P.scheme == 2) ? 2305843009213693952.0 : ldexp((double)P.n_slots, shift);
}

cudaError_t ws_launch_spacings(const WsScanParams& P, cudaStream_t s) {
    const int64_t n_all = P.n_slots + 1;
    const int64_t tiles = (n_all + WS_CDF_TILE - 1) / WS_CDF_TILE;
    int g = (int)(tiles < (int64_t)g_sm_count * 8 ? tiles : (int64_t)g_sm_count * 8);
    ws_spacing_tiles_kernel<<<g < 1 ? 1 : g, WS_SCAN_BLOCK, 0, s>>>(P);
    cudaError_t e = cudaGetLastError();
    if (e != cudaSuccess) return e;
    WsScanParams Q = P;
    Q.n = n_all;
    Q.tile_words = P.mn_tile_off;
    Q.total = P.mn_total;
    ws_cdf_offsets_kernel<<<1, 1024, 0, s>>>(Q);
    return cudaGetLastError();
}

cudaError_t ws_launch_cdf(const WsScanParams& P, cudaStream_t s) {
    const int64_t cdf_tiles = (P.n + WS_CDF_TILE - 1) / WS_CDF_TILE;
    int g1 = (int)(cdf_tiles < (int64_t)g_sm_count * WS_CDF_GRID ? cdf_tiles : (int64_t)g_sm_count * WS_CDF_GRID);
    if (g1 < 1) g1 = 1;
    ws_cdf_tiles_kernel<<<g1, WS_SCAN_BLOCK, 0, s>>>(P);
    cudaError_t e = cudaGetLastError();
    if (e != cudaSuccess) return e;
    ws_cdf_group_offsets_kernel<<<1, 1024, 0, s>>>(P);
    return cudaGetLastError();
}

cudaError_t ws_launch_bounds(const WsScanParams& P, cudaStream_t s) {
    const bool exact_fp = P.replay_u != nullptr || P.sorted_u != nullptr;
    if (exact_fp) ws_bounds_kernel<true><<<1, 32, 0, s>>>(P);
    else ws_bounds_kernel<false><<<1, 32, 0, s>>>(P);
    return cudaGetLastError();
}

cudaError_t ws_launch_cdf_tiles(const WsScanParams& P, cudaStream_t s) {
    const int64_t cdf_tiles = (P.n + WS_CDF_TILE - 1) / WS_CDF_TILE;
    int g1 = (int)(cdf_tiles < (int64_t)g_sm_count * WS_CDF_GRID ? cdf_tiles : (int64_t)g_sm_count * WS_CDF_GRID);
    if (g1 < 1) g1 = 1;
    ws_cdf_tiles_kernel<<<g1, WS_SCAN_BLOCK, 0, s>>>(P);
    return cudaGetLastError();
}
cudaError_t ws_launch_offsets_bounds_mbox(const WsScanParams& P, const WsMailbox& M, unsigned long long* all_tot, const unsigned long long* xmine,
                                          int xw, unsigned long long* xall, cudaStream_t s) {
    const bool exact_fp = P.replay_u != nullptr || P.sorted_u != nullptr;
    if (exact_fp) ws_offsets_bounds_mbox_kernel<true><<<1, 1024, 0, s>>>(P, M, all_tot, xmine, xw, xall);
    else ws_offsets_bounds_mbox_kernel<false><<<1, 1024, 0, s>>>(P, M, all_tot, xmine, xw, xall);
    return cudaGetLastError();
}

cudaError_t ws_launch_search(const WsScanParams& P, cudaStream_t s) {
    const int64_t warp_tiles = (P.n + WS_SCAN_TILE - 1) / WS_SCAN_TILE;
    const int64_t ctas = (warp_tiles + WS_WARPS_PER_CTA - 1) / WS_WARPS_PER_CTA;
    int g3 = (int)(ctas < (int64_t)g_sm_count * WS_SEARCH_GRID ? ctas : (int64_t)g_sm_count * WS_SEARCH_GRID);
    if (g3 < 1) g3 = 1;
    const bool exact_fp = P.replay_u != nullptr || P.sorted_u != nullptr;
    if (exact_fp) ws_search_kernel<true, false, false><<<g3, WS_SCAN_BLOCK, WS_SEARCH_SMEM_BYTES, s>>>(P);
    else if (P.scheme == 2) ws_search_kernel<false, true, false><<<g3, WS_SCAN_BLOCK, WS_SEARCH_SMEM_BYTES, s>>>(P);
    else if (P.fx_shift >= 32) ws_search_kernel<false, false, true><<<g3, WS_SCAN_BLOCK, WS_SEARCH_SMEM_BYTES, s>>>(P);
    else ws_search_kernel<false, false, false><<<g3, WS_SCAN_BLOCK, WS_SEARCH_SMEM_BYTES, s>>>(P);
    cudaError_t e = cudaGetLastError();
    if (e != cudaSuccess) return e;
    ws_expand_heavy_kernel<<<g_sm_count * 4, 256, 0, s>>>(P);
    return cudaGetLastError();
}

#ifndef WS_SCAN_DEFAULT_FORM
#define WS_SCAN_DEFAULT_FORM 0
#endif
static int g_scan_form = WS_SCAN_DEFAULT_FORM;
#ifndef WS_CHAIN_DEFAULT_BLOCK
#define WS_CHAIN_DEFAULT_BLOCK WS_SCAN_BLOCK
#endif
static int g_chain_block = WS_CHAIN_DEFAULT_BLOCK;
template <int BLOCK>
static cudaError_t ws_launch_chain(const WsScanParams& P, bool exact_fp, cudaStream_t s) {
    const int64_t tiles = (P.n + BLOCK * WS_SCAN_ITEMS - 1) / (BLOCK * WS_SCAN_ITEMS);
    const int64_t resident = (int64_t)g_sm_count * WS_CHAIN_MINB * (WS_SCAN_BLOCK / BLOCK);
    int g = (int)(tiles < resident ? tiles : resident);
    if (g < 1) g = 1;
    if (exact_fp) ws_chain_kernel<true, BLOCK><<<g, BLOCK, WS_CHAIN_SMEM_BYTES(BLOCK), s>>>(P);
    else ws_chain_kernel<false, BLOCK><<<g, BLOCK, WS_CHAIN_SMEM_BYTES(BLOCK), s>>>(P);
    return cudaGetLastError();
}
cudaError_t ws_launch_scan_search(const WsScanParams& P, int grid, cudaStream_t s) {
    (void)grid;
    if (g_scan_form != 0 && P.all_tot == nullptr && P.total == nullptr && P.bounds == nullptr && P.scheme != 2) {
        const int64_t cdf_tiles = (P.n + WS_CDF_TILE - 1) / WS_CDF_TILE;
        const bool exact_fp = P.replay_u != nullptr || P.sorted_u != nullptr;
        cudaError_t e = cudaMemsetAsync(P.tile_counter, 0, sizeof(unsigned int) * 2, s);
        if (e != cudaSuccess) return e;
        if (g_scan_form == 2) {
            const int64_t ch_tiles = (P.n + g_chain_block * WS_SCAN_ITEMS - 1) / (g_chain_block * WS_SCAN_ITEMS);
            e = cudaMemsetAsync(P.tile_words, 0, sizeof(unsigned long long) * (size_t)(ch_tiles + 3 * ((ch_tiles + WS_CHAIN_GROUP - 1) / WS_CHAIN_GROUP)), s);
            if (e != cudaSuccess) return e;
            e = g_chain_block == 32 ? ws_launch_chain<32>(P, exact_fp, s) : (g_chain_block == 64 ? ws_launch_chain<64>(P, exact_fp, s) : ws_launch_chain<WS_SCAN_BLOCK>(P, exact_fp, s));
            if (e != cudaSuccess) return e;
        } else {
            e = cudaMemsetAsync(P.tile_words, 0, sizeof(unsigned long long) * (size_t)cdf_tiles, s);
            if (e != cudaSuccess) return e;
            if (exact_fp) ws_scan_search_kernel<true><<<(unsigned)cdf_tiles, WS_SCAN_BLOCK, 0, s>>>(P);
            else ws_scan_search_kernel<false><<<(unsigned)cdf_tiles, WS_SCAN_BLOCK, 0, s>>>(P);
        }
        e = cudaGetLastError();
        if (e != cudaSuccess) return e;
        ws_expand_heavy_kernel<<<g_sm_count * 4, 256, 0, s>>>(P);
        return cudaGetLastError();
    }
    cudaError_t e = ws_launch_cdf(P, s);
    if (e != cudaSuccess) return e;
    return ws_launch_search(P, s);
}

__global__ void __launch_bounds__(256) ws_gather_kernel(const __grid_constant__ WsGatherParams P) {
    const int64_t stride = (int64_t)gridDim.x * 256;
    for (int64_t i = (int64_t)blockIdx.x * 256 + threadIdx.x; i < P.n; i += stride) {
        const int64_t a = (int64_t)__ldg(P.ancestors + i);
        for (int p0 = 0; p0 < P.n_planes; p0 += 8) {
            double v[8];
#pragma unroll
            for (int k = 0; k < 8; ++k)
                if (p0 + k < P.n_planes) v[k] = __ldg(P.src[p0 + k] + a);
#pragma unroll
            for (int k = 0; k < 8; ++k)
                if (p0 + k < P.n_planes) P.dst[p0 + k][i] = v[k];
        }
    }
}

cudaError_t ws_launch_gather(const WsGatherParams& P, int grid, cudaStream_t s) {
    ws_gather_kernel<<<grid, 256, 0, s>>>(P);
    return cudaGetLastError();
}

__global__ void ws_fill_kernel(double* __restrict__ dst, double v, int64_t n) {
    const int64_t stride = (int64_t)gridDim.x * blockDim.x;
    for (int64_t i = (int64_t)blockIdx.x * blockDim.x + threadIdx.x; i < n; i += stride) dst[i] = v;
}
cudaError_t ws_launch_fill(double* dst, double v, int64_t n, int grid, cudaStream_t s) {
    ws_fill_kernel<<<grid, 256, 0, s>>>(dst, v, n);
    return cudaGetLastError();
}

__global__ void ws_exp_norm_kernel(const double* __restrict__ logw, const WsReduceOut* __restrict__ red,
                                   double* __restrict__ w, int64_t n) {
    const double m = red->m, S = red->S;
    const double rS = 1.0 / S;
    const int64_t stride = (int64_t)gridDim.x * blockDim.x;
    for (int64_t i = (int64_t)blockIdx.x * blockDim.x + threadIdx.x; i < n; i += stride) w[i] = ws_div_pos(ws_exp_nonpos(logw[i] - m), S, rS);
}
cudaError_t ws_launch_exp_norm(const double* logw, const WsReduceOut* red, double* w, int64_t n, int grid,
                               cudaStream_t s) {
    ws_exp_norm_kernel<<<grid, 256, 0, s>>>(logw, red, w, n);
    return cudaGetLastError();
}

__global__ void __launch_bounds__(256) ws_sumsq_kernel(const double* __restrict__ w, int64_t n,
                                                       double* __restrict__ partials) {
    __shared__ double sc[8];
    double acc = 0.0;
    const int64_t stride = (int64_t)gridDim.x * 256;
    for (int64_t i = (int64_t)blockIdx.x * 256 + threadIdx.x; i < n; i += stride) {
        const double v = w[i];
        acc += v * v;
    }
#pragma unroll
    for (int d = 16; d > 0; d >>= 1) acc += __shfl_down_sync(0xffffffffu, acc, d);
    if ((threadIdx.x & 31) == 0) sc[threadIdx.x >> 5] = acc;
    __syncthreads();
    if (threadIdx.x == 0) {
        double t = 0.0;
        for (int k = 0; k < 8; ++k) t += sc[k];
        partials[blockIdx.x] = t;
    }
}
cudaError_t ws_launch_sumsq(const double* w, int64_t n, double* partials, int grid, cudaStream_t s) {
    ws_sumsq_kernel<<<grid, 256, 0, s>>>(w, n, partials);
    return cudaGetLastError();
}

__global__ void ws_local_ancestors_kernel(int32_t* __restrict__ anc, int64_t n, const int32_t* __restrict__ anc_self,
                                          int64_t self_lo, int64_t self_hi, int64_t spare_base) {
    const int64_t stride = (int64_t)gridDim.x * blockDim.x;
    for (int64_t i = (int64_t)blockIdx.x * blockDim.x + threadIdx.x; i < n; i += stride) {
        int32_t a;
        if (i < self_lo) a = (int32_t)(n + spare_base + i);
        else if (i >= self_hi) a = (int32_t)(n + spare_base + self_lo + (i - self_hi));
        else a = anc_self[i - self_lo];
        anc[i] = a;
    }
}
// ... 138 lines not shown
```

weightedsampling.jl_b200/csrc/ws_runtime.cu:

```cuda
#include <math.h>
#include <stdarg.h>
#include <stdio.h>
#include <string.h>
#include <algorithm>
#include <functional>
#include <memory>
#include <deque>
#include <map>
#include <string>
#include <vector>

#include <dlfcn.h>
#include <unistd.h>
#include <chrono>

#include "../../include/wsb200.h"
#include "ws_internal.h"
#include "ws_lowering.h"
#include "ws_move.h"
#include "ws_stats.h"
#include "ws_exchange.h"

using wsl::Plane;
using wsl::Program;
// ... 46 lines not shown
    WS_SYM(CommDestroy, "ncclCommDestroy")
    WS_SYM(AllGather, "ncclAllGather")
    WS_SYM(AllReduce, "ncclAllReduce")
    WS_SYM(Send, "ncclSend")
    WS_SYM(Recv, "ncclRecv")
    WS_SYM(GroupStart, "ncclGroupStart")
    WS_SYM(GroupEnd, "ncclGroupEnd")
    WS_SYM(GetErrorString, "ncclGetErrorString")
#undef WS_SYM
    g_nccl.handle = h;
    return true;
}

enum WsKernelClass { KC_VM = 0, KC_REDUCE, KC_FINALIZE, KC_SCAN, KC_GATHER, KC_FILL, KC_MOVE, KC_OTHER, KC_COUNT };

struct Column {
    std::string name;
    int32_t width;
    std::vector<double*> front, back;
    std::vector<uint8_t> stale;
    std::vector<int64_t> ep;
};

struct TimedEvent {
    int kclass;
    cudaEvent_t a, b;
};

struct TapeEntry {
    int64_t depth;
    int32_t op_end;
    int32_t cache_ops;
    double konst_end;
    std::function<void(Program&)> lower;
    std::vector<Plane> refs;
};

struct OwnedExprs {
    std::vector<std::vector<ws_tok>> toks;
    std::vector<ws_expr> ex;
    explicit OwnedExprs(std::initializer_list<std::pair<const ws_expr*, int>> groups) {
        for (auto& g : groups)
            for (int i = 0; i < g.second; ++i) toks.emplace_back(g.first[i].toks, g.first[i].toks + g.first[i].n);
        for (auto& t : toks) ex.push_back(ws_expr{t.data(), (int32_t)t.size(), 0});
    }
    void planes(std::vector<Plane>& out) const {
        for (auto& t : toks)
            for (auto& k : t)
                if (k.op == WS_TOK_PLANE) out.push_back(Plane{k.col, k.comp});
    }
};

struct ws_ctx {
    int device = 0;
    int sm_count = 148;
    cudaStream_t stream = nullptr;
    int64_t n = 0;
    int64_t spare = 0;
    int64_t n_global = 0;
    int64_t offset = 0;
    int rank = 0, nranks = 1;
    uint64_t seed = 0;
    uint64_t next_stream = 1;
    double ess_perc_min = 0.5;
    int resampler = WS_RESAMPLER_STRATIFIED;

    bool resampled = false, weights_changed = false;
    int64_t depth = 0;

    std::vector<Column> cols;
    std::map<std::string, int32_t> col_index;

    double* logw = nullptr;
    bool logw_uniform = true;
    double logw_base = 0.0;
    bool partials_valid = false;
    int n_partials = 0;
    WsLse* d_partials = nullptr;
    WsReduceOut* d_red = nullptr;
    WsReduceOut* h_red = nullptr;
    bool red_valid = false;
    static constexpr int SPEC_RING = 512;
    WsReduceOut* h_ring = nullptr;
    int64_t ring_event[SPEC_RING] = {0};
    int64_t spec_head = 0;
    int spec_pending = 0;
    bool logw_spec = false;
    bool async_resample = true;
    bool small_resample = true;
    ws_resample_info last_info{};
    bool last_info_pending = false;
    int spec_immediate = 0;
    struct SpecStep {
        size_t tape_size;
        Program::Mark score_mark;
        int64_t depth;
        uint64_t stream_before;
        int32_t ckpt_pc;
    };
    bool spec_block = false, spec_flushing = false;
    std::vector<SpecStep> spec_steps;
    double* d_logw_bak = nullptr;
    WsLse* d_ck_partials = nullptr;
    WsReduceOut* d_ck_red = nullptr;
    WsReduceOut* h_ck_red = nullptr;

    int32_t* d_anc = nullptr;
    bool anc_pending = false;
    struct AncVec {
        int64_t event;
        int32_t* ptr;
        bool identity = false;
    };
    int64_t epoch = 0;
    std::deque<AncVec> anc_live;
    std::vector<int32_t*> anc_pool;
    bool genealogy = true;
    size_t genealogy_budget = 0;
    std::vector<WsSpareRing> spare_rings;
    bool event_keeps = false;
    void* d_gen = nullptr;
    size_t gen_bytes = 0;
    int64_t traced_rows = 0;
    int64_t trace_forced_planes = 0, trace_full_gathers = 0, trace_ipc_rounds = 0;
    struct Slab {
        char* base;
        size_t size, used;
    };
    std::vector<Slab> slabs;
    int32_t* d_map = nullptr;
    int64_t map_ep = -1, map_E = -1;
    bool lazy_gather = true;
    unsigned long long* d_tile_words = nullptr;
    unsigned long long* d_cdf_local = nullptr;
    unsigned int* d_tile_counter = nullptr;
    int32_t* d_heavy_F = nullptr;
    unsigned long long* d_mn = nullptr;
    int64_t mn_cap_slots = 0;
    int64_t heavy_cap_n = 0;
    int64_t n_tiles = 0;
    unsigned long long* d_counters = nullptr;

    Program win;
    Program score;
    std::vector<TapeEntry> tape;
    WsOp* d_score_ops = nullptr;
    size_t d_score_cap = 0, d_score_uploaded = 0;
    WsOp* d_seg_ops = nullptr;
    size_t d_seg_cap = 0;
    bool record_only = false;
    bool tape_enabled = true;
    bool score_wide = false;

    double* d_replay_n = nullptr;
    double* d_replay_u = nullptr;
    double* d_replay_e = nullptr;
    double* d_replay_v = nullptr;
    int64_t replay_v_len = 0, cur_v = 0;
    int64_t replay_n_len = 0, replay_u_len = 0, replay_e_len = 0;
    int64_t cur_n = 0, cur_u = 0, cur_e = 0;

    double* d_scratch = nullptr;
    void* d_scratch2 = nullptr;
    size_t scratch2_bytes = 0;
    size_t scratch_bytes = 0;
    double* h_scratch = nullptr;
// ... 196 lines not shown
    c->score.temp_base = 0;
    c->score.n_temp_slots = WS_SCORE_TEMPS;
    c->score.max_regs = WS_SCORE_MAX_REGS;
    c->score.max_ops = 1 << 30;
    c->score.max_io = 1 << 30;
    c->tape.clear();
    c->d_score_uploaded = 0;
    c->score_wide = false;
}

extern "C" int ws_abi_version(void) { return WSB200_ABI_VERSION; }

extern "C" int ws_device_count(int* out) {
    int n = 0;
    cudaError_t e = cudaGetDeviceCount(&n);
    if (e != cudaSuccess) {
        if (out) *out = 0;
        return fail(nullptr, WS_ENODEVICE, "cudaGetDeviceCount: %s", cudaGetErrorString(e));
    }
    if (out) *out = n;
    return WS_OK;
}

extern "C" const char* ws_last_error(const ws_ctx* ctx) { return ctx ? ctx->err.c_str() : g_create_error.c_str(); }

extern "C" int ws_create_sharded(ws_ctx** out, int64_t n_global, int rank, int nranks, const void* nccl_unique_id,
                                 int device, uint64_t seed, double ess_perc_min, int resampler) {
    if (out == nullptr) return fail(nullptr, WS_EINVAL, "ws_create: out is NULL");
    *out = nullptr;
    if (n_global <= 0) return fail(nullptr, WS_EINVAL, "ws_create: n_particles must be positive (got %lld)", (long long)n_global);
    if (n_global >= (int64_t)2147483647 - 65536) return fail(nullptr, WS_EINVAL, "ws_create: n_particles must be < 2^31 - 65536 (Int32 ancestors)");
    if (nranks < 1 || rank < 0 || rank >= nranks) return fail(nullptr, WS_EINVAL, "ws_create: bad rank %d of %d", rank, nranks);
    if (nranks > 1 && nccl_unique_id == nullptr) return fail(nullptr, WS_EINVAL, "ws_create_sharded: nccl_unique_id is NULL");
    if (nranks > 1) {
        std::string err;
        if (!load_nccl(err)) return fail(nullptr, WS_ENCCL, "%s", err.c_str());
    }
    if (resampler < 0 || resampler > 2) return fail(nullptr, WS_EINVAL, "ws_create: unknown resampler %d", resampler);
    int ndev = 0;
    cudaError_t e = cudaGetDeviceCount(&ndev);
    if (e != cudaSuccess || ndev == 0)
        return fail(nullptr, WS_ENODEVICE, "no CUDA device available (%s); wsb200 has no CPU fallback",
                    e != cudaSuccess ? cudaGetErrorString(e) : "device count is 0");
    if (device < 0 || device >= ndev) return fail(nullptr, WS_EINVAL, "ws_create: device %d out of range (0..%d)", device, ndev - 1);

    ws_ctx* c = new ws_ctx();
    c->device = device;
    c->rank = rank;
    c->nranks = nranks;
    c->n_global = n_global;
    const int64_t lo = (n_global * rank) / nranks, hi = (n_global * (rank + 1)) / nranks;
    c->n = hi - lo;
    c->offset = lo;
    c->seed = seed;
    c->ess_perc_min = ess_perc_min;
    c->resampler = resampler;
    reset_window(c);
    reset_score(c);

#define CKC(call)                                                                                   \
    do {                                                                                            \
        cudaError_t e__ = (call);                                                                   \
        if (e__ != cudaSuccess) {                                                                   \
            int rc__ = fail(nullptr, e__ == cudaErrorMemoryAllocation ? WS_ENOMEM : WS_ECUDA, "%s failed: %s", #call, \
                            cudaGetErrorString(e__));                                               \
            ws_destroy(c);                                                                          \
            return rc__;                                                                            \
        }                                                                                           \
    } while (0)
    CKC(cudaSetDevice(device));
    cudaDeviceProp prop;
    CKC(cudaGetDeviceProperties(&prop, device));
    c->sm_count = prop.multiProcessorCount;
    CKC(ws_kernels_init(device));
    CKC(ws_move_kernels_init(device));
    CKC(ws_stats_init(device));
    CKC(cudaStreamCreateWithFlags(&c->stream, cudaStreamNonBlocking));
    CKC(cudaMalloc(&c->logw, sizeof(double) * (size_t)c->n));
    CKC(cudaMalloc(&c->d_partials, sizeof(WsLse) * WS_MAX_PARTIALS));
    CKC(cudaMalloc(&c->d_red, sizeof(WsReduceOut)));
    CKC(cudaMemsetAsync(c->d_red, 0, sizeof(WsReduceOut), c->stream));
    CKC(cudaMallocHost(&c->h_red, sizeof(WsReduceOut)));
    memset(c->h_red, 0, sizeof(WsReduceOut));
    CKC(cudaMallocHost(&c->h_ring, sizeof(WsReduceOut) * ws_ctx::SPEC_RING));
    {
        const char* v = getenv("WSB200_ASYNC_RESAMPLE");
        c->async_resample = !(v != nullptr && strcmp(v, "0") == 0);
        v = getenv("WSB200_SMALL_RESAMPLE");
        c->small_resample = !(v != nullptr && strcmp(v, "0") == 0);
    }
    if (nranks > 1) c->spare = std::max<int64_t>(4096, c->n / 32);
    if (pool_alloc(c, (void**)&c->d_anc, sizeof(int32_t) * (size_t)(c->n + 2 * c->spare)) != WS_OK) {
        int rc__ = fail(nullptr, WS_ENOMEM, "%s", c->err.c_str());
        ws_destroy(c);
        return rc__;
    }
    c->d_anc += c->spare;
    {
        size_t free_b = 0, total_b = 0;
        cudaMemGetInfo(&free_b, &total_b);
        c->genealogy_budget = total_b / 4;
        if (const char* e = getenv("WSB200_GENEALOGY_BYTES")) c->genealogy_budget = (size_t)strtoull(e, nullptr, 10);
        if (const char* e = getenv("WSB200_GENEALOGY")) c->genealogy = atoi(e) != 0;
    }
    c->n_tiles = (c->n + WS_CDF_TILE - 1) / WS_CDF_TILE;
    CKC(cudaMalloc(&c->d_tile_words, sizeof(unsigned long long) * ws_scan_words(c->n)));
    CKC(cudaMalloc(&c->d_cdf_local, sizeof(unsigned long long) * (size_t)c->n));
    CKC(cudaMalloc(&c->d_tile_counter, sizeof(unsigned int) * 2));
    CKC(cudaMalloc(&c->d_counters, sizeof(unsigned long long) * 4));
    CKC(cudaMemsetAsync(c->d_counters, 0, sizeof(unsigned long long) * 4, c->stream));
    CKC(cudaMalloc(&c->d_all_msq, sizeof(double) * 3 * (size_t)(nranks + 1)));
    CKC(cudaMalloc(&c->d_all_tot, sizeof(unsigned long long) * (size_t)(nranks + 1)));
    CKC(cudaMalloc(&c->d_all_bounds, sizeof(int32_t) * 2 * (size_t)(nranks + 1)));
#undef CKC
    if (nranks > 1) {
        ncclUniqueId id;
        memcpy(&id, nccl_unique_id, sizeof(id));
        int r = g_nccl.CommInitRank(&c->comm, nranks, id, rank);
        if (r != 0) {
            int rc = fail(nullptr, WS_ENCCL, "ncclCommInitRank failed: %s", g_nccl.GetErrorString(r));
            ws_destroy(c);
            return rc;
        }
        c->peer_slabs.resize((size_t)nranks);
        c->spare_rings.assign((size_t)nranks, WsSpareRing());
        if (const char* e = getenv("WSB200_EXCHANGE")) c->push_exchange = strcmp(e, "nccl") != 0;
        if (const char* e = getenv("WSB200_PUSH_MIN")) c->push_min = strtoll(e, nullptr, 10);
        if (cudaMalloc(&c->d_barrier, 64) != cudaSuccess || cudaMemset(c->d_barrier, 0, 64) != cudaSuccess) {
            int rc = fail(nullptr, WS_ECUDA, "cudaMalloc failed (barrier word)");
            ws_destroy(c);
            return rc;
        }
        {
            bool ok = g_nccl.GroupStart() == 0;
            for (int d = 0; d < nranks && ok; ++d) {
                if (d == rank) continue;
                ok = ok && g_nccl.Send(c->d_all_msq + 3 * nranks, 3, WS_NCCL_FLOAT64, d, c->comm, c->stream) == 0;
                ok = ok && g_nccl.Recv(c->d_all_msq + 3 * d, 3, WS_NCCL_FLOAT64, d, c->comm, c->stream) == 0;
            }
            ok = ok && g_nccl.GroupEnd() == 0;
            ok = ok && g_nccl.AllGather(c->d_all_tot + nranks, c->d_all_tot, 1, WS_NCCL_UINT64, c->comm, c->stream) == 0;
            ok = ok && g_nccl.AllReduce(c->d_all_msq, c->d_all_msq, 3, WS_NCCL_FLOAT64, WS_NCCL_SUM, c->comm, c->stream) == 0;
            if (!ok || cudaStreamSynchronize(c->stream) != cudaSuccess) {
                int rc = fail(nullptr, WS_ENCCL, "NCCL warm-up exchange failed");
                ws_destroy(c);
                return rc;
            }
        }
        if (mbox_setup(c) != WS_OK) {
            int rc = fail(nullptr, WS_ENCCL, "%s", c->err.c_str());
            ws_destroy(c);
            return rc;
        }
    }
    c->logw_uniform = true;
    c->logw_base = 0.0;
    *out = c;
    return WS_OK;
}

extern "C" int ws_create(ws_ctx** out, int64_t n_particles, int device, uint64_t seed, double ess_perc_min, int resampler) {
    return ws_create_sharded(out, n_particles, 0, 1, nullptr, device, seed, ess_perc_min, resampler);
}

extern "C" int ws_nccl_unique_id(void* out128) {
    if (out128 == nullptr) return fail(nullptr, WS_EINVAL, "ws_nccl_unique_id: out is NULL");
    std::string err;
    if (!load_nccl(err)) return fail(nullptr, WS_ENCCL, "%s", err.c_str());
    ncclUniqueId id;
    int r = g_nccl.GetUniqueId(&id);
    if (r != 0) return fail(nullptr, WS_ENCCL, "ncclGetUniqueId failed: %s", g_nccl.GetErrorString(r));
    memcpy(out128, &id, sizeof(id));
    return WS_OK;
}

extern "C" int ws_destroy(ws_ctx* c) {
    if (c == nullptr) return WS_OK;
    cudaSetDevice(c->device);
    if (c->stream) cudaStreamSynchronize(c->stream);
    if (getenv("WSB200_TRACE") && c->phase_n > 0)
        fprintf(stderr, "[wsb200 rank %d] sharded resample host ms/step: cdf+exchanges+sync %.3f | (of the exchange: peer addresses %.3f) | "
                        "search launch %.3f | exchange %.3f (steady %.3f) | (of the exchange: traced push %.3f) | of the first: plane addresses %.3f | prepare %.3f  (n=%lld)\n",
                c->rank, c->phase_ms[0] / c->phase_n, c->phase_ms[1] / c->phase_n, c->phase_ms[2] / c->phase_n,
                c->phase_ms[3] / c->phase_n, c->phase_ms[5] / std::max<int64_t>(1, c->phase_n - 6), c->phase_ms[4] / c->phase_n,
                c->phase_ms[6] / c->phase_n, c->phase_ms[7] / c->phase_n, (long long)c->phase_n);
    if (getenv("WSB200_TRACE") && c->phase_n > 0)
        fprintf(stderr, "[wsb200 rank %d] genealogy: %lld planes brought up to date to free vectors / spare rows, %lld events gathered everything, "
                        "%lld IPC mapping rounds, %zu slabs, traced values %lld\n",
                c->rank, (long long)c->trace_forced_planes, (long long)c->trace_full_gathers, (long long)c->trace_ipc_rounds, c->slabs.size(),
                (long long)c->traced_rows);
    if (c->d_scratch2) cudaFree(c->d_scratch2);
// ... 972 lines not shown
static int begin_resample_event(ws_ctx* c) {
    TRY(prepare_resample_event(c));
    return commit_resample_event(c);
}

static void end_resample_event(ws_ctx* c) {
    c->epoch++;
    for (auto& col : c->cols)
        for (auto& st : col.stale) st = 1;
    c->anc_pending = !c->cols.empty();
}

static int gather_all(ws_ctx* c, const int32_t* d_anc) {
    std::vector<Plane> which;
    for (int32_t ci = 0; ci < (int32_t)c->cols.size(); ++ci)
        for (int32_t k = 0; k < c->cols[ci].width; ++k) which.push_back(Plane{ci, k});
    return gather_planes(c, d_anc, which);
}

static bool small_resample_ok(const ws_ctx* c, const double* d_ru) {
    return c->small_resample && c->nranks == 1 && c->n <= WS_SMALL_N && d_ru == nullptr && c->resampler != WS_RESAMPLER_MULTINOMIAL;
}
static int run_small_resample(ws_ctx* c, uint64_t stream_id, int gate, int do_finalize) {
    WsScanParams S;
    memset(&S, 0, sizeof(S));
    S.logw = c->logw;
    S.mode = 0;
    S.scheme = c->resampler;
    S.red = c->d_red;
    S.gate = gate;
    S.n = c->n;
    S.n_slots = c->n;
    S.last_rank = 1;
    S.seed = c->seed;
    S.stream = stream_id;
    S.ancestors = c->d_anc;
    S.cdf_local = c->d_cdf_local;
    S.n_clamped = c->d_counters + 0;
    ws_scan_set_scale(S);
    TimedEvent te;
    timed_begin(c, KC_SCAN, te);
    CK(c, ws_launch_resample_small(S, c->d_partials, c->n_partials, c->ess_perc_min, c->d_red, c->d_counters + 3, do_finalize, c->stream));
    timed_end(c, te);
    return WS_OK;
}

static int prepare_multinomial(ws_ctx* c, WsScanParams& S) {
    const int64_t n_all = S.n_slots + 1;
    const int64_t tiles = (n_all + WS_CDF_TILE - 1) / WS_CDF_TILE, blocks = (n_all + WS_SCAN_TILE - 1) / WS_SCAN_TILE;
    if (c->d_mn == nullptr || c->mn_cap_slots < n_all) {
        if (c->d_mn) {
            CK(c, cudaStreamSynchronize(c->stream));
            CK(c, cudaFree(c->d_mn));
            c->d_mn = nullptr;
        }
        CK(c, cudaMalloc(&c->d_mn, sizeof(unsigned long long) * (size_t)(tiles + blocks + 2)));
        c->mn_cap_slots = n_all;
    }
    S.mn_tile_off = c->d_mn;
    S.mn_block_local = c->d_mn + tiles;
    S.mn_total = c->d_mn + tiles + blocks;
    TimedEvent te;
    timed_begin(c, KC_SCAN, te);
    CK(c, ws_launch_spacings(S, c->stream));
    timed_end(c, te);
    c->stats.kernel_launches += 1;
    return WS_OK;
}

static int sorted_replay_uniforms(ws_ctx* c, const double* d_ru, int64_t n, const double** d_sorted) {
    std::vector<double> u((size_t)n);
    CK(c, cudaMemcpyAsync(u.data(), d_ru, sizeof(double) * (size_t)n, cudaMemcpyDeviceToHost, c->stream));
    CK(c, cudaStreamSynchronize(c->stream));
    std::sort(u.begin(), u.end());
    TRY(ensure_scratch(c, sizeof(double) * (size_t)n));
    CK(c, cudaMemcpyAsync(c->d_scratch, u.data(), sizeof(double) * (size_t)n, cudaMemcpyHostToDevice, c->stream));
    CK(c, cudaStreamSynchronize(c->stream));
    *d_sorted = c->d_scratch;
    return WS_OK;
}

static int run_scan_search(ws_ctx* c, const double* d_w, int mode, int scheme, int64_t n, const double* d_replay_u,
                           const double* d_sorted_u, int32_t* d_anc, unsigned long long* d_words,
                           unsigned long long* d_cdf_local, uint64_t stream_id, unsigned long long* d_clamped, int gate = 0) {
    const int64_t n_tiles = (n + WS_CDF_TILE - 1) / WS_CDF_TILE;
    if (c->d_heavy_F == nullptr || c->heavy_cap_n < n) {
        if (c->d_heavy_F) {
            CK(c, cudaStreamSynchronize(c->stream));
            CK(c, cudaFree(c->d_heavy_F));
            c->d_heavy_F = nullptr;
        }
        const size_t slots = (size_t)(n / WS_HEAVY_TILE_SLOTS) + 2;
        CK(c, cudaMalloc(&c->d_heavy_F, sizeof(int32_t) * slots * (WS_SCAN_TILE + 2)));
        c->heavy_cap_n = n;
    }
    (void)n_tiles;
    WsScanParams S;
    memset(&S, 0, sizeof(S));
    S.logw = d_w;
    S.mode = mode;
    S.scheme = scheme;
    S.red = c->d_red;
    S.gate = gate;
    S.n = n;
    S.n_slots = n;
    S.cdf_offset = 0ull;
    S.slot_base = 0;
    S.last_rank = 1;
    S.bounds = nullptr;
    S.total = nullptr;
    S.seed = c->seed;
    S.stream = stream_id;
    S.replay_u = d_replay_u;
    S.sorted_u = d_sorted_u;
    S.ancestors = d_anc;
    S.tile_words = d_words;
    S.cdf_local = d_cdf_local;
    S.tile_counter = c->d_tile_counter;
    S.n_clamped = d_clamped;
    S.heavy_count = c->d_tile_counter + 1;
    S.heavy_F = c->d_heavy_F;
    ws_scan_set_scale(S);
    if (scheme == WS_RESAMPLER_MULTINOMIAL && d_sorted_u == nullptr && d_replay_u == nullptr) TRY(prepare_multinomial(c, S));
    TimedEvent te;
    timed_begin(c, KC_SCAN, te);
    CK(c, ws_launch_scan_search(S, 0, c->stream));
    c->stats.kernel_launches += 3;
    timed_end(c, te);
    return WS_OK;
}

static int allgather_host_bytes(ws_ctx* c, const void* mine, size_t bytes, std::vector<char>& all) {
    const size_t R = (size_t)c->nranks, words = bytes / 8;
    TRY(ensure_scratch2(c, bytes * (R + 1)));
    char* d = (char*)c->d_scratch2;
    CK(c, cudaMemcpyAsync(d + bytes * R, mine, bytes, cudaMemcpyHostToDevice, c->stream));
    NCK(c, g_nccl.AllGather(d + bytes * R, d, words, WS_NCCL_UINT64, c->comm, c->stream));
    all.resize(bytes * R);
    CK(c, cudaMemcpyAsync(all.data(), d, bytes * R, cudaMemcpyDeviceToHost, c->stream));
    CK(c, cudaStreamSynchronize(c->stream));
    return WS_OK;
}

static WsMailbox mbox_next(ws_ctx* c, int n_exchanges) {
    WsMailbox M;
    memset(&M, 0, sizeof(M));
    for (int q = 0; q < c->nranks; ++q) M.box[q] = c->mbox_peer[(size_t)q];
    M.rank = c->rank;
    M.nranks = c->nranks;
    M.seq = c->mbox_seq + 1u;
    M.cap = c->mbox_cap;
    M.err = c->d_mbox_err;
    M.timeout_ns = 60000000000ull;
    if (const char* e = getenv("WSB200_MAILBOX_TIMEOUT_MS")) M.timeout_ns = strtoull(e, nullptr, 10) * 1000000ull;
    c->mbox_seq += (uint32_t)n_exchanges;
    c->mbox_exchanges += n_exchanges;
    return M;
}
static int mbox_check(ws_ctx* c) {
    if (c->h_mbox_err != nullptr && *reinterpret_cast<volatile unsigned int*>(c->h_mbox_err) != 0u)
        return fail(c, WS_ENCCL, "mailbox exchange timed out: a rank died or the ranks left lock-step");
    return WS_OK;
}
static void mbox_release(ws_ctx* c) {
    for (size_t q = 0; q < c->mbox_peer.size(); ++q)
        if ((int)q != c->rank && c->mbox_peer[q]) cudaIpcCloseMemHandle(c->mbox_peer[q]);
    c->mbox_peer.clear();
    if (c->d_mbox) cudaFree(c->d_mbox);
    c->d_mbox = nullptr;
    c->mbox_on = false;
    cudaGetLastError();
}
static int mbox_setup(ws_ctx* c) {
    const int R = c->nranks, r = c->rank;
    if (const char* e = getenv("WSB200_MAILBOX"))
        if (strcmp(e, "0") == 0) return WS_OK;
    if (R > WS_MBOX_MAX_RANKS) return WS_OK;
    CK(c, cudaSetDevice(c->device));
    struct Msg {
        int64_t pid, ok;
        cudaIpcMemHandle_t h;
    };
    static_assert(sizeof(Msg) % 8 == 0, "Msg travels as 64-bit words");
    Msg mine;
    memset(&mine, 0, sizeof(mine));
    mine.pid = (int64_t)getpid();
    c->mbox_cap = 16384;
    const size_t bytes = sizeof(unsigned long long) * 2 * (size_t)R * (size_t)c->mbox_cap;
    bool ok = cudaMalloc(&c->d_mbox, bytes) == cudaSuccess && cudaMemset(c->d_mbox, 0, bytes) == cudaSuccess;
    if (ok && c->h_mbox_err == nullptr) {
        ok = cudaHostAlloc(&c->h_mbox_err, 64, cudaHostAllocMapped) == cudaSuccess;
        if (ok) {
            memset(c->h_mbox_err, 0, 64);
            ok = cudaHostGetDevicePointer((void**)&c->d_mbox_err, c->h_mbox_err, 0) == cudaSuccess;
        }
    }
    ok = ok && cudaIpcGetMemHandle(&mine.h, c->d_mbox) == cudaSuccess;
    ok = ok && cudaDeviceSynchronize() == cudaSuccess;
    cudaGetLastError();
    mine.ok = ok ? 1 : 0;
    std::vector<char> all;
    TRY(allgather_host_bytes(c, &mine, sizeof(mine), all));
    const Msg* msgs = reinterpret_cast<const Msg*>(all.data());
    bool usable = true;
    for (int q = 0; q < R; ++q) {
        if (!msgs[q].ok) usable = false;
        for (int q2 = q + 1; q2 < R; ++q2)
            if (msgs[q].pid == msgs[q2].pid) usable = false;
    }
    if (!usable) {
// ... 509 lines not shown
        info->resampled = c->resampled ? 1 : 0;
        info->ess_perc = NAN;
        info->log_mean_w = NAN;
        info->n_clamped = -1;
    }
    if (!c->weights_changed) {
        c->last_info = ws_resample_info{0, -1, NAN, NAN, -1};
        c->last_info_pending = false;
        return WS_OK;
    }
    if (c->resampler == WS_RESAMPLER_MULTINOMIAL && c->nranks > 1 && c->d_replay_u != nullptr)
        return fail(c, WS_EUNSUPPORTED, "multinomial resampling of a sharded state with replayed uniforms (Philox draws are supported)");
    const bool merged = c->nranks > 1 && c->d_replay_u == nullptr;
    TRY(ensure_reduced(c, true, !merged));
    c->stats.resamples_fired++;
    const uint64_t step_stream = c->next_stream++;
    int fired = 0;
    if (merged && !c->red_valid) {
        const auto tp0 = std::chrono::steady_clock::now();
        TRY(prepare_resample_event(c));
        c->phase_ms[7] += std::chrono::duration<double, std::milli>(std::chrono::steady_clock::now() - tp0).count();
        TRY(resample_sharded(c, nullptr, step_stream, &fired));
    } else if (c->h_red->do_resample) {
        fired = 1;
        const double* d_ru = nullptr;
        if (c->d_replay_u != nullptr) {
            const int64_t need = (c->resampler == WS_RESAMPLER_SYSTEMATIC) ? 1 : c->n_global;
            if (c->cur_u + need > c->replay_u_len)
                return fail(c, WS_EREPLAY, "replay uniforms exhausted in Resample (%lld needed, %lld installed)",
                            (long long)(c->cur_u + need), (long long)c->replay_u_len);
            d_ru = c->d_replay_u + c->cur_u;
            c->cur_u += need;
        }
        TRY(begin_resample_event(c));
        if (c->nranks > 1) {
            TRY(resample_sharded(c, d_ru, step_stream));
        } else {
            const double* d_sorted = nullptr;
            if (c->resampler == WS_RESAMPLER_MULTINOMIAL && d_ru != nullptr) {
                TRY(sorted_replay_uniforms(c, d_ru, c->n, &d_sorted));
                d_ru = nullptr;
            }
            if (small_resample_ok(c, d_ru) && d_sorted == nullptr) {
                TRY(run_small_resample(c, step_stream, 0, 0));
            } else {
                TRY(run_scan_search(c, c->logw, 0, c->resampler, c->n, d_ru, d_sorted, c->d_anc, c->d_tile_words, c->d_cdf_local, step_stream, c->d_counters + 0));
            }
            end_resample_event(c);
            if (!c->lazy_gather) TRY(materialize_planes(c));
        }
    }
    book_step(c, *c->h_red, fired != 0);
    if (info) *info = c->last_info;
    return WS_OK;
}

extern "C" int ws_resample_async(ws_ctx* c) {
    if (!c) return WS_EINVAL;
    if (c->spec_block && !c->spec_flushing) return spec_checkpoint(c);
    if (!c->weights_changed || !c->async_resample || c->d_replay_u != nullptr || c->nranks > 1 || c->resampler == WS_RESAMPLER_MULTINOMIAL ||
        !c->lazy_gather || c->cols.empty() || c->spec_immediate >= 2)
        return ws_resample(c, nullptr);
    TRY(flush_window(c));
    if (c->red_valid || c->logw_uniform || c->logw_spec) return ws_resample(c, nullptr);
    CK(c, cudaSetDevice(c->device));
    if (c->spec_pending >= ws_ctx::SPEC_RING - 1) TRY(resolve_spec(c));
    if (!c->partials_valid) {
        const int grid = std::min(grid_for(c, c->n, 256, 8), WS_MAX_PARTIALS);
        TimedEvent te;
        timed_begin(c, KC_REDUCE, te);
        CK(c, ws_launch_reduce_logw(c->logw, c->n, c->d_partials, grid, c->stream));
        timed_end(c, te);
        c->n_partials = grid;
        c->partials_valid = true;
    }
    const uint64_t stream_id = c->next_stream++;
    if (small_resample_ok(c, nullptr)) {
        TRY(begin_resample_event(c));
        TRY(run_small_resample(c, stream_id, 1, 1));
        CK(c, cudaMemcpyAsync(&c->h_ring[c->spec_head % ws_ctx::SPEC_RING], c->d_red, sizeof(WsReduceOut), cudaMemcpyDeviceToHost, c->stream));
        c->ring_event[c->spec_head % ws_ctx::SPEC_RING] = c->epoch + 1;
        end_resample_event(c);
    } else {
        TimedEvent te;
        timed_begin(c, KC_FINALIZE, te);
        CK(c, ws_launch_finalize(c->d_partials, c->n_partials, 1, c->n_global, c->ess_perc_min, c->d_red, c->d_counters + 3, c->stream));
        timed_end(c, te);
        CK(c, cudaMemcpyAsync(&c->h_ring[c->spec_head % ws_ctx::SPEC_RING], c->d_red, sizeof(WsReduceOut), cudaMemcpyDeviceToHost, c->stream));
        c->ring_event[c->spec_head % ws_ctx::SPEC_RING] = c->epoch + 1;
        TRY(begin_resample_event(c));
        TRY(run_scan_search(c, c->logw, 0, c->resampler, c->n, nullptr, nullptr, c->d_anc, c->d_tile_words, c->d_cdf_local, stream_id,
                            c->d_counters + 0, 1));
        end_resample_event(c);
    }
    c->spec_head++;
    c->spec_pending++;
    c->stats.resamples_fired++;
    c->logw_uniform = false;
    c->logw_spec = true;
    c->partials_valid = false;
    c->red_valid = false;
    c->weights_changed = false;
    c->last_info_pending = true;
    return WS_OK;
}

extern "C" int ws_exec(ws_ctx* c, const ws_cmd* cmds, int32_t n_cmds, const double* params, int32_t n_params) {
    if (!c || (!cmds && n_cmds > 0) || n_cmds < 0) return WS_EINVAL;
    std::vector<ws_tok> toks;
    std::vector<ws_expr> ex;
    for (int32_t k = 0; k < n_cmds; ++k) {
        const ws_cmd& cm = cmds[k];
        toks.clear();
        ex.clear();
        size_t first[3] = {0, 0, 0};
        std::vector<size_t> off;
        for (int a = 0; a < 3; ++a) {
            first[a] = ex.size();
            if (cm.n_e[a] < 0 || (cm.n_e[a] > 0 && cm.e[a] == nullptr)) return fail(c, WS_EINVAL, "ws_exec: command %d has a bad expression list", k);
            for (int32_t j = 0; j < cm.n_e[a]; ++j) {
                const ws_expr& src = cm.e[a][j];
                if (src.toks == nullptr || src.n <= 0) return fail(c, WS_EINVAL, "ws_exec: command %d has an empty expression", k);
                off.push_back(toks.size());
                for (int32_t i = 0; i < src.n; ++i) {
                    ws_tok t = src.toks[i];
                    if (t.op == WS_TOK_PARAM) {
                        if (t.col < 0 || t.col >= n_params || params == nullptr)
                            return fail(c, WS_EINVAL, "ws_exec: parameter %d of %d", t.col, n_params);
                        t.op = WS_TOK_CONST;
                        t.val = params[t.col];
                        t.col = 0;
                    }
                    toks.push_back(t);
                }
                ex.push_back(ws_expr{nullptr, src.n, 0});
            }
        }
        for (size_t j = 0; j < ex.size(); ++j) ex[j].toks = toks.data() + off[j];
        const ws_expr* e0 = cm.n_e[0] > 0 ? &ex[first[0]] : nullptr;
        const ws_expr* e1 = cm.n_e[1] > 0 ? &ex[first[1]] : nullptr;
        const ws_expr* e2 = cm.n_e[2] > 0 ? &ex[first[2]] : nullptr;
        switch (cm.fn) {
            case WS_CMD_ASSIGN: TRY(ws_assign(c, cm.i0, cm.i1, e0)); break;
            case WS_CMD_ASSIGN_VEC: TRY(ws_assign_vec(c, cm.i0, cm.i1, e0)); break;
            case WS_CMD_SAMPLE_NORMAL: TRY(ws_sample_normal(c, cm.i0, cm.i1, e0, e1)); break;
            case WS_CMD_SAMPLE_EXPONENTIAL: TRY(ws_sample_exponential(c, cm.i0, cm.i1, e0)); break;
            case WS_CMD_SAMPLE_MVNORMAL: TRY(ws_sample_mvnormal(c, cm.i0, cm.i1, e0, cm.mat)); break;
            case WS_CMD_OBSERVE_NORMAL: TRY(ws_observe_normal(c, e0, e1, e2)); break;
            case WS_CMD_OBSERVE_EXPONENTIAL: TRY(ws_observe_exponential(c, e0, e1)); break;
            case WS_CMD_OBSERVE_MVNORMAL: TRY(ws_observe_mvnormal(c, cm.i0, e0, e1, cm.mat)); break;
            case WS_CMD_WEIGHT_EXPR: TRY(ws_weight_expr(c, e0)); break;
            case WS_CMD_SAMPLE_EXPR: TRY(ws_sample_expr(c, cm.i0, cm.i1, e0, e1, e2)); break;
            case WS_CMD_RESAMPLE: TRY(ws_resample_async(c)); break;
            default: return fail(c, WS_EINVAL, "ws_exec: unknown command %d", cm.fn);
        }
    }
    return WS_OK;
}

extern "C" int ws_exec_n(ws_ctx* c, const ws_cmd* cmds, int32_t n_cmds, const double* params, int32_t n_params, int32_t n_elems) {
    if (!c || n_elems < 0 || (n_params > 0 && n_elems > 0 && !params)) return WS_EINVAL;
    for (int32_t e = 0; e < n_elems; ++e) TRY(ws_exec(c, cmds, n_cmds, params + (size_t)e * (size_t)n_params, n_params));
    return WS_OK;
}

static int spec_checkpoint(ws_ctx* c) {
    if (!c->weights_changed) return WS_OK;
    if (c->win.ops.empty() || !c->win.has_acc) return fail(c, WS_EUNSUPPORTED, "speculative block: a step without a weighting term");
    if (!c->win.dirty.empty()) return fail(c, WS_EUNSUPPORTED, "speculative block: a statement writes a column");
    if (c->spec_steps.size() >= WS_VM_MAX_CKPT) return fail(c, WS_EUNSUPPORTED, "speculative block: more than %d steps", WS_VM_MAX_CKPT);
    if (c->win.ops.size() > 255) return fail(c, WS_EUNSUPPORTED, "speculative block: window too long");
    ws_ctx::SpecStep st;
    st.tape_size = c->tape.size();
    st.score_mark = c->score.mark();
    st.depth = c->depth;
// ... 196 lines not shown
    }
};

static int reduce_host_array(ws_ctx* c, const double* d_logw, int64_t n) {
    TRY(resolve_spec(c));
    const int grid = std::min(grid_for(c, n, 256, 8), WS_MAX_PARTIALS);
    TimedEvent te;
    timed_begin(c, KC_REDUCE, te);
    CK(c, ws_launch_reduce_logw(d_logw, n, c->d_partials, grid, c->stream));
    timed_end(c, te);
    timed_begin(c, KC_FINALIZE, te);
    CK(c, ws_launch_finalize(c->d_partials, grid, 1, n, c->ess_perc_min, c->d_red, nullptr, c->stream));
    timed_end(c, te);
    CK(c, cudaMemcpyAsync(c->h_red, c->d_red, sizeof(WsReduceOut), cudaMemcpyDeviceToHost, c->stream));
    CK(c, cudaStreamSynchronize(c->stream));
    c->red_valid = false;
    c->partials_valid = false;
    return WS_OK;
}

extern "C" int ws_exp_norm_host(ws_ctx* c, const double* logw, int64_t n, double* w_out) {
    if (!c || !logw || !w_out || n <= 0) return c ? fail(c, WS_EINVAL, "ws_exp_norm_host: bad arguments") : WS_EINVAL;
    TRY(flush_window(c));
    CK(c, cudaSetDevice(c->device));
    TempBuf in, out;
    CK(c, cudaMalloc(&in.p, sizeof(double) * (size_t)n));
    CK(c, cudaMalloc(&out.p, sizeof(double) * (size_t)n));
    CK(c, cudaMemcpyAsync(in.p, logw, sizeof(double) * (size_t)n, cudaMemcpyHostToDevice, c->stream));
    TRY(reduce_host_array(c, (const double*)in.p, n));
    CK(c, ws_launch_exp_norm((const double*)in.p, c->d_red, (double*)out.p, n, grid_for(c, n, 256, 8), c->stream));
    c->stats.kernel_launches++;
    CK(c, cudaMemcpyAsync(w_out, out.p, sizeof(double) * (size_t)n, cudaMemcpyDeviceToHost, c->stream));
    CK(c, cudaStreamSynchronize(c->stream));
    c->stats.h2d_bytes += (int64_t)sizeof(double) * n;
    c->stats.d2h_bytes += (int64_t)sizeof(double) * n;
    return WS_OK;
}

extern "C" int ws_logsumexp_host(ws_ctx* c, const double* logw, int64_t n, double* out) {
    if (!c || !logw || !out || n <= 0) return c ? fail(c, WS_EINVAL, "ws_logsumexp_host: bad arguments") : WS_EINVAL;
    TRY(flush_window(c));
    CK(c, cudaSetDevice(c->device));
    TempBuf in;
    CK(c, cudaMalloc(&in.p, sizeof(double) * (size_t)n));
    CK(c, cudaMemcpyAsync(in.p, logw, sizeof(double) * (size_t)n, cudaMemcpyHostToDevice, c->stream));
    TRY(reduce_host_array(c, (const double*)in.p, n));
    *out = c->h_red->lse;
    c->stats.h2d_bytes += (int64_t)sizeof(double) * n;
    return WS_OK;
}

extern "C" int ws_ess_perc_host(ws_ctx* c, const double* w, int64_t n, double* out) {
    if (!c || !w || !out || n <= 0) return c ? fail(c, WS_EINVAL, "ws_ess_perc_host: bad arguments") : WS_EINVAL;
    TRY(flush_window(c));
    CK(c, cudaSetDevice(c->device));
    TempBuf in, part;
    const int grid = std::min(grid_for(c, n, 256, 8), WS_MAX_PARTIALS);
    CK(c, cudaMalloc(&in.p, sizeof(double) * (size_t)n));
    CK(c, cudaMalloc(&part.p, sizeof(double) * (size_t)grid));
    CK(c, cudaMemcpyAsync(in.p, w, sizeof(double) * (size_t)n, cudaMemcpyHostToDevice, c->stream));
    CK(c, ws_launch_sumsq((const double*)in.p, n, (double*)part.p, grid, c->stream));
    c->stats.kernel_launches++;
    std::vector<double> hp(grid);
    CK(c, cudaMemcpyAsync(hp.data(), part.p, sizeof(double) * (size_t)grid, cudaMemcpyDeviceToHost, c->stream));
    CK(c, cudaStreamSynchronize(c->stream));
    double s = 0.0;
    for (int i = 0; i < grid; ++i) s += hp[i];
    *out = 1.0 / ((double)n * s);
    c->stats.h2d_bytes += (int64_t)sizeof(double) * n;
    return WS_OK;
}

static int resample_host_impl(ws_ctx* c, const double* weights, int64_t n, int scheme, const double* uniforms,
                              int64_t n_uniforms, bool sorted_mode, int32_t* indices_out, int64_t* n_clamped) {
    TRY(flush_window(c));
    TRY(resolve_spec(c));
    CK(c, cudaSetDevice(c->device));
    if (n >= (int64_t)2147483647 - 65536) return fail(c, WS_EINVAL, "n must be < 2^31 - 65536");
    TempBuf w, u, anc, words, cdf;
    const int64_t n_tiles = (n + WS_CDF_TILE - 1) / WS_CDF_TILE;
    CK(c, cudaMalloc(&w.p, sizeof(double) * (size_t)n));
    CK(c, cudaMalloc(&anc.p, sizeof(int32_t) * (size_t)n));
    CK(c, cudaMalloc(&words.p, sizeof(unsigned long long) * ws_scan_words(n)));
    CK(c, cudaMalloc(&cdf.p, sizeof(unsigned long long) * (size_t)n));
    CK(c, cudaMemcpyAsync(w.p, weights, sizeof(double) * (size_t)n, cudaMemcpyHostToDevice, c->stream));
    if (uniforms != nullptr) {
        CK(c, cudaMalloc(&u.p, sizeof(double) * (size_t)n_uniforms));
        CK(c, cudaMemcpyAsync(u.p, uniforms, sizeof(double) * (size_t)n_uniforms, cudaMemcpyHostToDevice, c->stream));
    }
    CK(c, cudaMemsetAsync(c->d_counters + 1, 0, sizeof(unsigned long long), c->stream));
    const uint64_t stream_id = c->next_stream++;
    TRY(run_scan_search(c, (const double*)w.p, 1, scheme, n, sorted_mode ? nullptr : (const double*)u.p,
                        sorted_mode ? (const double*)u.p : nullptr, (int32_t*)anc.p, (unsigned long long*)words.p,
                        (unsigned long long*)cdf.p, stream_id, c->d_counters + 1));
    CK(c, cudaMemcpyAsync(indices_out, anc.p, sizeof(int32_t) * (size_t)n, cudaMemcpyDeviceToHost, c->stream));
    unsigned long long h_clamped = 0;
    CK(c, cudaMemcpyAsync(&h_clamped, c->d_counters + 1, sizeof(h_clamped), cudaMemcpyDeviceToHost, c->stream));
    CK(c, cudaStreamSynchronize(c->stream));
    if (n_clamped) *n_clamped = (int64_t)h_clamped;
    c->stats.h2d_bytes += (int64_t)sizeof(double) * (n + (uniforms ? n_uniforms : 0));
    c->stats.d2h_bytes += (int64_t)sizeof(int32_t) * n;
    return WS_OK;
}

extern "C" int ws_icdf_host(ws_ctx* c, const double* weights, const double* us, int64_t n, int32_t* indices_out, int64_t* n_clamped) {
    if (!c || !weights || !us || !indices_out || n <= 0) return c ? fail(c, WS_EINVAL, "ws_icdf_host: bad arguments") : WS_EINVAL;
    return resample_host_impl(c, weights, n, WS_RESAMPLER_STRATIFIED, us, n, true, indices_out, n_clamped);
}

extern "C" int ws_resample_host(ws_ctx* c, const double* weights, int64_t n, int scheme, const double* uniforms,
                                int32_t* indices_out, int64_t* n_clamped) {
    if (!c || !weights || !indices_out || n <= 0) return c ? fail(c, WS_EINVAL, "ws_resample_host: bad arguments") : WS_EINVAL;
    if (scheme == WS_RESAMPLER_STRATIFIED) return resample_host_impl(c, weights, n, scheme, uniforms, n, false, indices_out, n_clamped);
    if (scheme == WS_RESAMPLER_SYSTEMATIC) return resample_host_impl(c, weights, n, scheme, uniforms, 1, false, indices_out, n_clamped);
    if (scheme == WS_RESAMPLER_MULTINOMIAL) {
        if (uniforms == nullptr) return resample_host_impl(c, weights, n, scheme, nullptr, 0, false, indices_out, n_clamped);
        std::vector<double> su(uniforms, uniforms + n);
        std::sort(su.begin(), su.end());
        return resample_host_impl(c, weights, n, scheme, su.data(), n, true, indices_out, n_clamped);
    }
    return fail(c, WS_EINVAL, "unknown resampling scheme %d", scheme);
}

extern "C" int ws_expectation(ws_ctx* c, const ws_expr* f, int32_t n_exprs, double* out) {
    if (!c || !f || !out) return WS_EINVAL;
    if (n_exprs < 1 || n_exprs > 8) return fail(c, WS_EINVAL, "ws_expectation: 1..8 expressions per call");
    for (int k = 0; k < n_exprs; ++k) TRY(check_expr(c, &f[k], "ws_expectation"));
    TRY(ensure_reduced(c));
    Program p;
    p.max_regs = WS_VM_MAX_REGS;
    p.max_ops = WS_VM_MAX_OPS;
    p.max_io = WS_VM_MAX_IO;
    int regs[8];
    for (int k = 0; k < n_exprs; ++k) {
        Val v = p.compile(f[k]);
        int t = p.alloc_plane_reg();
        if (v.is_const)
            p.emit(ws_make_op(WS_OP_LIN2, t, WS_REG_NONE, WS_REG_NONE, WS_REG_NONE, 0, v.c0, 0, 0));
        else
            p.emit(ws_make_op(WS_OP_LIN2, t, v.reg, WS_REG_NONE, WS_REG_NONE, 0, v.c0, v.c1, 0));
        regs[k] = t;
        p.end_statement();
    }
    if (!p.error.empty()) return fail(c, WS_EINVAL, "%s", p.error.c_str());
    if (p.overflow) return fail(c, WS_EUNSUPPORTED, "ws_expectation: expressions do not fit one device pass");
    WsVmProgram P;
    memset(&P, 0, sizeof(P));
    P.n = c->n;
    P.particle_offset = c->offset;
    P.n_ops = (int)p.ops.size();
    P.n_loads = (int)p.loads.size();
    P.n_stores = 0;
    P.n_regs = std::max(1, p.high_water);
    {
        std::vector<Plane> loaded;
        for (auto& ld : p.loads) loaded.push_back(ld.first);
        TRY(materialize_deep(c, loaded));
    }
    P.ancestors = c->d_anc;
    for (int k = 0; k < P.n_loads; ++k) {
        const Plane pl = p.loads[k].first;
        P.load_ptr[k] = plane_ptr(c, pl);
        P.load_reg[k] = (uint8_t)p.loads[k].second;
        if (c->cols[pl.col].stale[pl.comp]) P.load_gather |= (1u << k);
    }
    P.logw_mode = 0;
// ... 864 lines not shown
```

Baseline: 44.92 billion.

## Fuse finalize and group offsets into CDF tile kernel and enable PDL launches

Folds the ESS finalize reduction into the CDF tiles kernel, where every block recombines the partials and block 0 writes the decision to device memory and to a mapped host ring. The separate 1024-thread group-offsets kernel is replaced by a last-block tail that accumulates group sums atomically. Launches for the VM, CDF, search and expand kernels now use programmatic dependent launch so each kernel's prologue can overlap the previous one. This removes two kernel launches and a D2H copy per resample, at the cost of redundant per-block partial combines, extra atomics, and zero-initialization requirements on the scratch buffers.

```diff
diff --git a/weightedsampling.jl_b200/csrc/ws_internal.h b/weightedsampling.jl_b200/csrc/ws_internal.h
--- a/weightedsampling.jl_b200/csrc/ws_internal.h
+++ b/weightedsampling.jl_b200/csrc/ws_internal.h
@@ -97,6 +97,13 @@
     unsigned long long* n_clamped;
     unsigned int* heavy_count;
     int32_t* heavy_F;
+    int32_t offsets_tail;
+    int32_t n_partials;
+    unsigned int* done_counter;
+    const WsLse* partials;
+    double ess_perc_min;
+    unsigned long long* ties;
+    WsReduceOut* red_host;
 };
 
 struct WsGatherParams {
@@ -125,8 +132,8 @@
 cudaError_t ws_launch_resample_small(const WsScanParams& P, const WsLse* partials, int n_partials, double ess_perc_min, WsReduceOut* out,
                                      unsigned long long* ties, int do_finalize, cudaStream_t s);
 void ws_scan_set_scale(WsScanParams& P);
-size_t ws_scan_words(int64_t n);
-cudaError_t ws_launch_scan_search(const WsScanParams& P, int grid, cudaStream_t s);
+__host__ __device__ size_t ws_scan_words(int64_t n);
+cudaError_t ws_launch_scan_search(const WsScanParams& P, int* n_kernels, cudaStream_t s);
 cudaError_t ws_launch_spacings(const WsScanParams& P, cudaStream_t s);
 cudaError_t ws_launch_cdf(const WsScanParams& P, cudaStream_t s);
 cudaError_t ws_launch_bounds(const WsScanParams& P, cudaStream_t s);
diff --git a/weightedsampling.jl_b200/csrc/ws_kernels.cu b/weightedsampling.jl_b200/csrc/ws_kernels.cu
--- a/weightedsampling.jl_b200/csrc/ws_kernels.cu
+++ b/weightedsampling.jl_b200/csrc/ws_kernels.cu
@@ -117,6 +117,23 @@
     out->log_mean_w = lse - log(nn);
     out->do_resample = (out->ess_perc < ess_perc_min) ? 1 : 0;
     if (ties != nullptr && fabs(out->ess_perc - ess_perc_min) <= 8.0 * 2.220446049250313e-16 * fabs(ess_perc_min)) atomicAdd(ties, 1ull);
+}
+
+__device__ __forceinline__ void ws_pdl_wait() { asm volatile("griddepcontrol.wait;" ::: "memory"); }
+
+template <typename... KArgs, typename... Args>
+static cudaError_t ws_launch_pdl(void (*kernel)(KArgs...), unsigned grid, unsigned block, size_t smem, cudaStream_t s, Args... args) {
+    cudaLaunchAttribute attr[1];
+    attr[0].id = cudaLaunchAttributeProgrammaticStreamSerialization;
+    attr[0].val.programmaticStreamSerializationAllowed = 1;
+    cudaLaunchConfig_t cfg = {};
+    cfg.gridDim = dim3(grid);
+    cfg.blockDim = dim3(block);
+    cfg.dynamicSmemBytes = smem;
+    cfg.stream = s;
+    cfg.attrs = attr;
+    cfg.numAttrs = 1;
+    return cudaLaunchKernelEx(&cfg, kernel, args...);
 }
 
 __device__ __forceinline__ void ws_cp_async8(double* smem_dst, const double* gsrc) {
@@ -381,6 +398,10 @@
     part.Q = 0.0;
     const int n = (int)P.n;
     const int n_tiles = (n + TILE - 1) / TILE;
+    WsSlConsts<Sig> K;
+    ws_sl_load_consts<Sig>(K, P, std::make_integer_sequence<int, Sig::n_ops>{});
+    const bool replay = P.rng.replay_n != nullptr || P.rng.replay_u != nullptr || P.rng.replay_e != nullptr;
+    ws_pdl_wait();
     const bool fired = (P.logw_mode != 3) || P.red->do_resample != 0;
     const int lmode = (P.logw_mode == 3) ? (fired ? 2 : 1) : P.logw_mode;
     const double lbase = (P.logw_mode == 3) ? P.red->log_mean_w : P.logw_base;
@@ -401,10 +422,6 @@
         }
         ws_cp_async_commit();
     };
-
-    WsSlConsts<Sig> K;
-    ws_sl_load_consts<Sig>(K, P, std::make_integer_sequence<int, Sig::n_ops>{});
-    const bool replay = P.rng.replay_n != nullptr || P.rng.replay_u != nullptr || P.rng.replay_e != nullptr;
 
     int anc_next[PP];
     {
@@ -598,8 +615,7 @@
     int grid = (int)(tiles < (int64_t)g_sm_count * WS_SL_MINB ? tiles : (int64_t)g_sm_count * WS_SL_MINB);
     if (grid < 1) grid = 1;
     const int smem = (Sig::n_loads > 0 ? Sig::n_loads : 1) * TILE * (int)sizeof(double);
-    ws_vm_sl_kernel<Sig, WS_SL_P><<<grid, WS_VM_BLOCK, smem, s>>>(P);
-    return cudaGetLastError();
+    return ws_launch_pdl(ws_vm_sl_kernel<Sig, WS_SL_P>, (unsigned)grid, WS_VM_BLOCK, (size_t)smem, s, P);
 }
 int ws_vm_sl_grid(const WsVmProgram& P) {
     if (!g_vm_interp_only && P.n_ckpt != 0 && ws_slck_ok(P)) return ws_slck_grid(P);
@@ -826,19 +842,61 @@
 #ifndef WS_CDF_GRID
 #define WS_CDF_GRID 4
 #endif
+__device__ void ws_cdf_offsets_tail(const WsScanParams& P, int n_tiles, unsigned long long* gsum);
+__device__ __forceinline__ void ws_fence_acq_rel() { asm volatile("fence.acq_rel.gpu;" ::: "memory"); }
+#ifndef WS_CDF_DIAG
+#define WS_CDF_DIAG 0
+#endif
+#if WS_CDF_DIAG
+#include <cstdio>
+__device__ unsigned long long g_cdf_diag[4];
+#endif
 __global__ void __launch_bounds__(WS_SCAN_BLOCK, WS_CDF_MINB) ws_cdf_tiles_kernel(const __grid_constant__ WsScanParams P) {
-    if (P.gate != 0 && P.red->do_resample == 0) return;
     __shared__ unsigned long long warp_tot[2][WS_SCAN_BLOCK / 32];
+    ws_pdl_wait();
     int parity = 0;
     const int lane = threadIdx.x & 31, warp = threadIdx.x >> 5;
     const int n = (int)P.n;
     const int n_tiles = (n + WS_CDF_TILE - 1) / WS_CDF_TILE;
-    double m = 0.0, Sden = 1.0;
-    if (P.mode == 0) {
-        m = P.red->m;
-        Sden = P.red->S;
-    }
-    const double rS = 1.0 / Sden;
+    unsigned long long* const gsum = P.tile_words + ws_scan_words(n) - (n_tiles + WS_TILE_GROUP - 1) / WS_TILE_GROUP;
+    double m = 0.0, Sden = 1.0, rS = 1.0;
+    __shared__ WsLse warp_scratch[WS_SCAN_BLOCK / 32];
+    __shared__ double s_m, s_S;
+    __shared__ int s_fire;
+#if WS_CDF_DIAG
+    if (blockIdx.x == 0 && threadIdx.x == 0) g_cdf_diag[0] = ws_globaltimer();
+#endif
+    auto closed = [&]() -> bool {
+        if (P.partials != nullptr) {
+            const WsLse tot = lse_block_combine<WS_SCAN_BLOCK>(P.partials, P.n_partials, warp_scratch);
+            if (threadIdx.x == 0) {
+                WsReduceOut d;
+                ws_decide(tot, P.n_slots, P.ess_perc_min, &d, blockIdx.x == 0 ? P.ties : nullptr);
+                if (blockIdx.x == 0) {
+                    *const_cast<WsReduceOut*>(P.red) = d;
+                    *P.red_host = d;
+                }
+                s_m = d.m;
+                s_S = d.S;
+                s_fire = d.do_resample;
+            }
+            __syncthreads();
+            if (P.gate != 0 && s_fire == 0) return true;
+            m = s_m;
+            Sden = s_S;
+        } else {
+            if (P.gate != 0 && P.red->do_resample == 0) return true;
+            if (P.mode == 0) {
+                m = P.red->m;
+                Sden = P.red->S;
+            }
+        }
+        rS = 1.0 / Sden;
+#if WS_CDF_DIAG
+        if (blockIdx.x == 0 && threadIdx.x == 0) g_cdf_diag[1] = ws_globaltimer();
+#endif
+        return false;
+    };
     const double uniform_w = 1.0 / (double)P.n_slots;
 #if WS_CDF_ASYNC
     __shared__ __align__(16) double2 lbuf_all[WS_SCAN_ITEMS / 2][WS_SCAN_BLOCK];
@@ -851,6 +909,7 @@
         }
         ws_cp_async_commit();
     };
+    if (closed()) return;
     if ((int)blockIdx.x < n_tiles) request(blockIdx.x);
     for (int tile = blockIdx.x; tile < n_tiles; tile += gridDim.x) {
         const int item0 = tile * WS_CDF_TILE + threadIdx.x * WS_SCAN_ITEMS;
@@ -902,6 +961,7 @@
 #pragma unroll
     for (int k = 0; k < WS_SCAN_ITEMS; ++k) l[k] = -INFINITY;
     if (P.mode != 2 && (int)blockIdx.x < n_tiles) load_tile(blockIdx.x, l);
+    if (closed()) return;
     for (int tile = blockIdx.x; tile < n_tiles; tile += gridDim.x) {
         const int item0 = tile * WS_CDF_TILE + threadIdx.x * WS_SCAN_ITEMS;
         unsigned long long q[WS_SCAN_ITEMS];
@@ -952,18 +1012,23 @@
             for (int k = 0; k < WS_SCAN_ITEMS; ++k)
                 if (item0 + k < n) P.cdf_local[item0 + k] = thread_excl + q[k];
         }
-        if (threadIdx.x == 0) P.tile_words[tile] = tile_agg;
-    }
+        if (threadIdx.x == 0) {
+            P.tile_words[tile] = tile_agg;
+            if (P.offsets_tail) atomicAdd(gsum + tile / WS_TILE_GROUP, tile_agg);
+        }
+    }
+    if (P.offsets_tail) ws_cdf_offsets_tail(P, n_tiles, gsum);
 }
 
 #define WS_OFF_ITEMS 8
+template <int BLOCK>
 __device__ __forceinline__ void ws_scan_words_cta(unsigned long long* __restrict__ words, const int n_tiles, unsigned long long* total_out) {
-    __shared__ unsigned long long warp_tot[32];
+    __shared__ unsigned long long warp_tot[BLOCK / 32];
     __shared__ unsigned long long s_carry;
     const int lane = threadIdx.x & 31, warp = threadIdx.x >> 5;
     if (threadIdx.x == 0) s_carry = 0ull;
     __syncthreads();
-    for (int base = 0; base < n_tiles; base += 1024 * WS_OFF_ITEMS) {
+    for (int base = 0; base < n_tiles; base += BLOCK * WS_OFF_ITEMS) {
         const int i0 = base + threadIdx.x * WS_OFF_ITEMS;
         unsigned long long v[WS_OFF_ITEMS];
 #pragma unroll
@@ -981,7 +1046,7 @@
         __syncthreads();
         unsigned long long warp_excl = 0ull, total = 0ull;
 #pragma unroll
-        for (int w = 0; w < 32; ++w) {
+        for (int w = 0; w < BLOCK / 32; ++w) {
             const unsigned long long t = warp_tot[w];
             if (w < warp) warp_excl += t;
             total += t;
@@ -1001,7 +1066,7 @@
 }
 __global__ void __launch_bounds__(1024) ws_cdf_offsets_kernel(const __grid_constant__ WsScanParams P) {
     if (P.gate != 0 && P.red->do_resample == 0) return;
-    ws_scan_words_cta(P.tile_words, (int)((P.n + WS_CDF_TILE - 1) / WS_CDF_TILE), P.total);
+    ws_scan_words_cta<1024>(P.tile_words, (int)((P.n + WS_CDF_TILE - 1) / WS_CDF_TILE), P.total);
 }
 __device__ __forceinline__ void ws_cdf_group_offsets_body(const WsScanParams& P) {
     if (threadIdx.x == 0 && P.heavy_count != nullptr) *P.heavy_count = 0u;
@@ -1018,9 +1083,40 @@
         if (lane == 0) grp[g] = v;
     }
     __syncthreads();
-    ws_scan_words_cta(grp, n_groups, P.total);
-}
-__global__ void __launch_bounds__(1024) ws_cdf_group_offsets_kernel(const __grid_constant__ WsScanParams P) { ws_cdf_group_offsets_body(P); }
+    ws_scan_words_cta<1024>(grp, n_groups, P.total);
+}
+__device__ void ws_cdf_offsets_tail(const WsScanParams& P, const int n_tiles, unsigned long long* const gsum) {
+    __shared__ int s_last;
+    if (threadIdx.x == 0) {
+        ws_fence_acq_rel();
+        s_last = atomicAdd(P.done_counter, 1u) == gridDim.x - 1;
+        if (s_last) {
+#if WS_CDF_DIAG
+            g_cdf_diag[2] = ws_globaltimer();
+#endif
+            ws_fence_acq_rel();
+            *P.done_counter = 0u;
+            if (P.heavy_count != nullptr) *P.heavy_count = 0u;
+        }
+    }
+    __syncthreads();
+    if (!s_last) return;
+    const int n_groups = (n_tiles + WS_TILE_GROUP - 1) / WS_TILE_GROUP;
+    unsigned long long* const grp = P.tile_words + n_tiles;
+    for (int g = threadIdx.x; g < n_groups; g += WS_SCAN_BLOCK) {
+        grp[g] = __ldcg(gsum + g);
+        gsum[g] = 0ull;
+    }
+    __syncthreads();
+    ws_scan_words_cta<WS_SCAN_BLOCK>(grp, n_groups, P.total);
+#if WS_CDF_DIAG
+    if (threadIdx.x == 0) {
+        const unsigned long long t3 = ws_globaltimer();
+        printf("CDFDIAG prologue_ns %llu tail_start_ns %llu tail_ns %llu total_ns %llu\n", g_cdf_diag[1] - g_cdf_diag[0],
+               g_cdf_diag[2] - g_cdf_diag[0], t3 - g_cdf_diag[2], t3 - g_cdf_diag[0]);
+    }
+#endif
+}
 __device__ __forceinline__ unsigned long long ws_tile_offset(const WsScanParams& P, const int n_tiles, const int ct, const int lane) {
     const int g = ct / WS_TILE_GROUP, idx = g * WS_TILE_GROUP + lane;
     unsigned long long v = idx < ct ? __ldg(P.tile_words + idx) : 0ull;
@@ -1595,6 +1691,7 @@
 #define WS_SEARCH_SMEM_BYTES ((WS_WARPS_PER_CTA * WS_RBUF_SLOTS + WS_CDF_TILE) * 8)
 template <bool EXACT_FP, bool MN, bool SHR>
 __global__ void __launch_bounds__(WS_SCAN_BLOCK, WS_SEARCH_MINB) ws_search_kernel(const __grid_constant__ WsScanParams P) {
+    ws_pdl_wait();
     if (ws_gate_closed_identity(P)) return;
 
     extern __shared__ __align__(16) unsigned long long search_smem[];
@@ -1835,10 +1932,11 @@
 #define WS_CHAIN_SMEM_BYTES(BLOCK) ((((BLOCK) / 32) * WS_RBUF_SLOTS + 2 * (BLOCK) * WS_SCAN_ITEMS) * 8)
 #define WS_CHAIN_MIN_TILE (32 * WS_SCAN_ITEMS)
 
-size_t ws_scan_words(int64_t n) {
+__host__ __device__ size_t ws_scan_words(int64_t n) {
     const int64_t n_tiles = (n + WS_CHAIN_MIN_TILE - 1) / WS_CHAIN_MIN_TILE;
     const int64_t n_groups = (n_tiles + WS_CHAIN_GROUP - 1) / WS_CHAIN_GROUP;
-    return (size_t)(n_tiles + 3 * n_groups + 2);
+    const int64_t cdf_groups = ((n + WS_CDF_TILE - 1) / WS_CDF_TILE + WS_TILE_GROUP - 1) / WS_TILE_GROUP;
+    return (size_t)(n_tiles + 3 * n_groups + 2 + cdf_groups);
 }
 
 template <bool EXACT_FP, int BLOCK>
@@ -2157,6 +2255,7 @@
 }
 
 __global__ void __launch_bounds__(256) ws_expand_heavy_kernel(const __grid_constant__ WsScanParams P) {
+    ws_pdl_wait();
     if (P.gate != 0 && P.red->do_resample == 0) return;
     __shared__ int32_t Fs[WS_SCAN_TILE];
     const unsigned int n_heavy = *P.heavy_count;
@@ -2217,15 +2316,16 @@
     return cudaGetLastError();
 }
 
-cudaError_t ws_launch_cdf(const WsScanParams& P, cudaStream_t s) {
+cudaError_t ws_launch_cdf_tiles(const WsScanParams& P, cudaStream_t s) {
     const int64_t cdf_tiles = (P.n + WS_CDF_TILE - 1) / WS_CDF_TILE;
     int g1 = (int)(cdf_tiles < (int64_t)g_sm_count * WS_CDF_GRID ? cdf_tiles : (int64_t)g_sm_count * WS_CDF_GRID);
     if (g1 < 1) g1 = 1;
-    ws_cdf_tiles_kernel<<<g1, WS_SCAN_BLOCK, 0, s>>>(P);
-    cudaError_t e = cudaGetLastError();
-    if (e != cudaSuccess) return e;
-    ws_cdf_group_offsets_kernel<<<1, 1024, 0, s>>>(P);
-    return cudaGetLastError();
+    return ws_launch_pdl(ws_cdf_tiles_kernel, (unsigned)g1, WS_SCAN_BLOCK, 0, s, P);
+}
+cudaError_t ws_launch_cdf(const WsScanParams& P, cudaStream_t s) {
+    WsScanParams Q = P;
+    Q.offsets_tail = 1;
+    return ws_launch_cdf_tiles(Q, s);
 }
 
 cudaError_t ws_launch_bounds(const WsScanParams& P, cudaStream_t s) {
@@ -2235,13 +2335,6 @@
     return cudaGetLastError();
 }
 
-cudaError_t ws_launch_cdf_tiles(const WsScanParams& P, cudaStream_t s) {
-    const int64_t cdf_tiles = (P.n + WS_CDF_TILE - 1) / WS_CDF_TILE;
-    int g1 = (int)(cdf_tiles < (int64_t)g_sm_count * WS_CDF_GRID ? cdf_tiles : (int64_t)g_sm_count * WS_CDF_GRID);
-    if (g1 < 1) g1 = 1;
-    ws_cdf_tiles_kernel<<<g1, WS_SCAN_BLOCK, 0, s>>>(P);
-    return cudaGetLastError();
-}
 cudaError_t ws_launch_offsets_bounds_mbox(const WsScanParams& P, const WsMailbox& M, unsigned long long* all_tot, const unsigned long long* xmine,
                                           int xw, unsigned long long* xall, cudaStream_t s) {
     const bool exact_fp = P.replay_u != nullptr || P.sorted_u != nullptr;
@@ -2256,14 +2349,13 @@
     int g3 = (int)(ctas < (int64_t)g_sm_count * WS_SEARCH_GRID ? ctas : (int64_t)g_sm_count * WS_SEARCH_GRID);
     if (g3 < 1) g3 = 1;
     const bool exact_fp = P.replay_u != nullptr || P.sorted_u != nullptr;
-    if (exact_fp) ws_search_kernel<true, false, false><<<g3, WS_SCAN_BLOCK, WS_SEARCH_SMEM_BYTES, s>>>(P);
-    else if (P.scheme == 2) ws_search_kernel<false, true, false><<<g3, WS_SCAN_BLOCK, WS_SEARCH_SMEM_BYTES, s>>>(P);
-    else if (P.fx_shift >= 32) ws_search_kernel<false, false, true><<<g3, WS_SCAN_BLOCK, WS_SEARCH_SMEM_BYTES, s>>>(P);
-    else ws_search_kernel<false, false, false><<<g3, WS_SCAN_BLOCK, WS_SEARCH_SMEM_BYTES, s>>>(P);
-    cudaError_t e = cudaGetLastError();
+    auto search = exact_fp ? ws_search_kernel<true, false, false>
+                : P.scheme == 2 ? ws_search_kernel<false, true, false>
+                : P.fx_shift >= 32 ? ws_search_kernel<false, false, true>
+                : ws_search_kernel<false, false, false>;
+    cudaError_t e = ws_launch_pdl(search, (unsigned)g3, WS_SCAN_BLOCK, WS_SEARCH_SMEM_BYTES, s, P);
     if (e != cudaSuccess) return e;
-    ws_expand_heavy_kernel<<<g_sm_count * 4, 256, 0, s>>>(P);
-    return cudaGetLastError();
+    return ws_launch_pdl(ws_expand_heavy_kernel, (unsigned)(g_sm_count * 4), 256, 0, s, P);
 }
 
 #ifndef WS_SCAN_DEFAULT_FORM
@@ -2284,12 +2376,19 @@
     else ws_chain_kernel<false, BLOCK><<<g, BLOCK, WS_CHAIN_SMEM_BYTES(BLOCK), s>>>(P);
     return cudaGetLastError();
 }
-cudaError_t ws_launch_scan_search(const WsScanParams& P, int grid, cudaStream_t s) {
-    (void)grid;
+cudaError_t ws_launch_scan_search(const WsScanParams& P, int* n_kernels, cudaStream_t s) {
     if (g_scan_form != 0 && P.all_tot == nullptr && P.total == nullptr && P.bounds == nullptr && P.scheme != 2) {
         const int64_t cdf_tiles = (P.n + WS_CDF_TILE - 1) / WS_CDF_TILE;
         const bool exact_fp = P.replay_u != nullptr || P.sorted_u != nullptr;
-        cudaError_t e = cudaMemsetAsync(P.tile_counter, 0, sizeof(unsigned int) * 2, s);
+        *n_kernels = 2;
+        cudaError_t e;
+        if (P.partials != nullptr) {
+            ws_finalize_kernel<<<1, 256, 0, s>>>(P.partials, P.n_partials, P.n_slots, P.ess_perc_min, const_cast<WsReduceOut*>(P.red), P.ties);
+            e = cudaMemcpyAsync(P.red_host, P.red, sizeof(WsReduceOut), cudaMemcpyDefault, s);
+            if (e != cudaSuccess) return e;
+            *n_kernels = 3;
+        }
+        e = cudaMemsetAsync(P.tile_counter, 0, sizeof(unsigned int) * 2, s);
         if (e != cudaSuccess) return e;
         if (g_scan_form == 2) {
             const int64_t ch_tiles = (P.n + g_chain_block * WS_SCAN_ITEMS - 1) / (g_chain_block * WS_SCAN_ITEMS);
@@ -2308,6 +2407,7 @@
         ws_expand_heavy_kernel<<<g_sm_count * 4, 256, 0, s>>>(P);
         return cudaGetLastError();
     }
+    *n_kernels = 3;
     cudaError_t e = ws_launch_cdf(P, s);
     if (e != cudaSuccess) return e;
     return ws_launch_search(P, s);
diff --git a/weightedsampling.jl_b200/csrc/ws_runtime.cu b/weightedsampling.jl_b200/csrc/ws_runtime.cu
--- a/weightedsampling.jl_b200/csrc/ws_runtime.cu
+++ b/weightedsampling.jl_b200/csrc/ws_runtime.cu
@@ -152,6 +152,7 @@
     bool red_valid = false;
     static constexpr int SPEC_RING = 512;
     WsReduceOut* h_ring = nullptr;
+    WsReduceOut* d_ring = nullptr;
     int64_t ring_event[SPEC_RING] = {0};
     int64_t spec_head = 0;
     int spec_pending = 0;
@@ -514,7 +515,8 @@
     CKC(cudaMemsetAsync(c->d_red, 0, sizeof(WsReduceOut), c->stream));
     CKC(cudaMallocHost(&c->h_red, sizeof(WsReduceOut)));
     memset(c->h_red, 0, sizeof(WsReduceOut));
-    CKC(cudaMallocHost(&c->h_ring, sizeof(WsReduceOut) * ws_ctx::SPEC_RING));
+    CKC(cudaHostAlloc(&c->h_ring, sizeof(WsReduceOut) * ws_ctx::SPEC_RING, cudaHostAllocMapped));
+    CKC(cudaHostGetDevicePointer(&c->d_ring, c->h_ring, 0));
     {
         const char* v = getenv("WSB200_ASYNC_RESAMPLE");
         c->async_resample = !(v != nullptr && strcmp(v, "0") == 0);
@@ -537,8 +539,10 @@
     }
     c->n_tiles = (c->n + WS_CDF_TILE - 1) / WS_CDF_TILE;
     CKC(cudaMalloc(&c->d_tile_words, sizeof(unsigned long long) * ws_scan_words(c->n)));
+    CKC(cudaMemsetAsync(c->d_tile_words, 0, sizeof(unsigned long long) * ws_scan_words(c->n), c->stream));
     CKC(cudaMalloc(&c->d_cdf_local, sizeof(unsigned long long) * (size_t)c->n));
-    CKC(cudaMalloc(&c->d_tile_counter, sizeof(unsigned int) * 2));
+    CKC(cudaMalloc(&c->d_tile_counter, sizeof(unsigned int) * 3));
+    CKC(cudaMemsetAsync(c->d_tile_counter, 0, sizeof(unsigned int) * 3, c->stream));
     CKC(cudaMalloc(&c->d_counters, sizeof(unsigned long long) * 4));
     CKC(cudaMemsetAsync(c->d_counters, 0, sizeof(unsigned long long) * 4, c->stream));
     CKC(cudaMalloc(&c->d_all_msq, sizeof(double) * 3 * (size_t)(nranks + 1)));
@@ -1677,7 +1681,8 @@
 
 static int run_scan_search(ws_ctx* c, const double* d_w, int mode, int scheme, int64_t n, const double* d_replay_u,
                            const double* d_sorted_u, int32_t* d_anc, unsigned long long* d_words,
-                           unsigned long long* d_cdf_local, uint64_t stream_id, unsigned long long* d_clamped, int gate = 0) {
+                           unsigned long long* d_cdf_local, uint64_t stream_id, unsigned long long* d_clamped, int gate = 0,
+                           WsReduceOut* record = nullptr) {
     const int64_t n_tiles = (n + WS_CDF_TILE - 1) / WS_CDF_TILE;
     if (c->d_heavy_F == nullptr || c->heavy_cap_n < n) {
         if (c->d_heavy_F) {
@@ -1715,12 +1720,21 @@
     S.n_clamped = d_clamped;
     S.heavy_count = c->d_tile_counter + 1;
     S.heavy_F = c->d_heavy_F;
+    S.done_counter = c->d_tile_counter + 2;
+    if (record != nullptr) {
+        S.partials = c->d_partials;
+        S.n_partials = c->n_partials;
+        S.ess_perc_min = c->ess_perc_min;
+        S.ties = c->d_counters + 3;
+        S.red_host = record;
+    }
     ws_scan_set_scale(S);
     if (scheme == WS_RESAMPLER_MULTINOMIAL && d_sorted_u == nullptr && d_replay_u == nullptr) TRY(prepare_multinomial(c, S));
     TimedEvent te;
     timed_begin(c, KC_SCAN, te);
-    CK(c, ws_launch_scan_search(S, 0, c->stream));
-    c->stats.kernel_launches += 3;
+    int n_kernels = 0;
+    CK(c, ws_launch_scan_search(S, &n_kernels, c->stream));
+    c->stats.kernel_launches += n_kernels - 1;
     timed_end(c, te);
     return WS_OK;
 }
@@ -2396,15 +2410,10 @@
         c->ring_event[c->spec_head % ws_ctx::SPEC_RING] = c->epoch + 1;
         end_resample_event(c);
     } else {
-        TimedEvent te;
-        timed_begin(c, KC_FINALIZE, te);
-        CK(c, ws_launch_finalize(c->d_partials, c->n_partials, 1, c->n_global, c->ess_perc_min, c->d_red, c->d_counters + 3, c->stream));
-        timed_end(c, te);
-        CK(c, cudaMemcpyAsync(&c->h_ring[c->spec_head % ws_ctx::SPEC_RING], c->d_red, sizeof(WsReduceOut), cudaMemcpyDeviceToHost, c->stream));
         c->ring_event[c->spec_head % ws_ctx::SPEC_RING] = c->epoch + 1;
         TRY(begin_resample_event(c));
         TRY(run_scan_search(c, c->logw, 0, c->resampler, c->n, nullptr, nullptr, c->d_anc, c->d_tile_words, c->d_cdf_local, stream_id,
-                            c->d_counters + 0, 1));
+                            c->d_counters + 0, 1, &c->d_ring[c->spec_head % ws_ctx::SPEC_RING]));
         end_resample_event(c);
     }
     c->spec_head++;
@@ -2767,6 +2776,7 @@
     CK(c, cudaMalloc(&w.p, sizeof(double) * (size_t)n));
     CK(c, cudaMalloc(&anc.p, sizeof(int32_t) * (size_t)n));
     CK(c, cudaMalloc(&words.p, sizeof(unsigned long long) * ws_scan_words(n)));
+    CK(c, cudaMemsetAsync(words.p, 0, sizeof(unsigned long long) * ws_scan_words(n), c->stream));
     CK(c, cudaMalloc(&cdf.p, sizeof(unsigned long long) * (size_t)n));
     CK(c, cudaMemcpyAsync(w.p, weights, sizeof(double) * (size_t)n, cudaMemcpyHostToDevice, c->stream));
     if (uniforms != nullptr) {
```

After: 45.71 billion (median of 6 runs). +1.8%, better.
